# suous/RecNeXt

Measured on AMD Instinct MI355X. Metric: images/sec RecNeXt-M3 224x224 bf16, higher is better.
Workload: dtype bf16

## Files before the change

include/recnext_amd.h:

```cpp
#ifndef RECNEXT_AMD_H
#define RECNEXT_AMD_H

#include <stddef.h>

#ifdef __cplusplus
extern "C" {
#endif

#define RCX_ABI_VERSION 7

enum { RCX_DTYPE_F32 = 0, RCX_DTYPE_BF16 = 1, RCX_DTYPE_F16 = 2 };
enum { RCX_MODE_BILINEAR = 0, RCX_MODE_NEAREST = 1 };
enum { RCX_MAX_LEVEL = 8 };

enum {
    RCX_ERR_BAD_ARG = -1,
    RCX_ERR_UNSUPPORTED = -2,
    RCX_ERR_WORKSPACE = -3
};

int rcx_abi_version(void);
const char* rcx_last_error(void);
void rcx_reload_options(void);

int rcx_selftest_d16(const void* src, void* flag, void* stream);

const char* rcx_recconv2d_fwd_plan(int N, int C, int H, int W, int level, int k, int mode, int dtype);

int rcx_pack_dw_weight(const void* w_ckk, float* dst_kkc, int C, int k, int dtype, void* stream);
int rcx_pack_recconv_params(const void* const* w, const void* const* b, float* wpack, float* wpack_flipped, float* bpack,
                            int count, int C, int k, int dtype, void* stream);
int rcx_unpack_recconv_grads(const float* gwpack, void* const* gw, int count, int C, int k, void* stream);
int rcx_pack_bias(const void* b, float* dst, int C, int dtype, void* stream);

size_t rcx_recconv2d_fwd_workspace_bytes(int N, int C, int H, int W, int level, int k, int dtype);

int rcx_recconv2d_fwd(const void* x, void* y, const float* wpack, const float* bpack,
                      void* workspace, size_t workspace_bytes,
                      int N, int C, int H, int W, int level, int k, int mode, int dtype, void* stream);

int rcx_time_next_launch(void* start_event, void* stop_event);
int rcx_launch_events_pending(void);

size_t rcx_recconv2d_train_saved_bytes(int N, int C, int H, int W, int level, int k);
size_t rcx_recconv2d_bwd_workspace_bytes(int N, int C, int H, int W, int level, int k);
int rcx_recconv2d_fwd_train(const void* x, void* y, const float* wpack, const float* bpack, void* saved, size_t saved_bytes,
                            int N, int C, int H, int W, int level, int k, int mode, int dtype, void* stream);
int rcx_recconv2d_bwd_gy_dtype(int N, int C, int H, int W, int level, int k, int dtype);
const char* rcx_recconv2d_bwd_plan(int N, int C, int H, int W, int level, int k, int dtype);
int rcx_recconv2d_bwd(const void* x, const void* gy, int gy_dtype, const float* wpack, const float* wpack_flipped, const void* saved,
                      void* gx, float* gwpack, float* gbpack, void* const* gw_out, void* const* gb_out, int grad_dtype,
                      void* workspace, size_t workspace_bytes,
                      int N, int C, int H, int W, int level, int k, int mode, int dtype, void* stream);

size_t rcx_recconv2d_bwd_input_workspace_bytes(int N, int C, int H, int W, int level, int k);
int rcx_recconv2d_bwd_input_gy_dtype(int N, int C, int H, int W, int level, int k, int dtype);
const char* rcx_recconv2d_bwd_input_plan(int N, int C, int H, int W, int level, int k, int dtype);
int rcx_recconv2d_bwd_input(const void* gy, int gy_dtype, const float* wpack, const float* wpack_flipped, void* gx,
                            void* workspace, size_t workspace_bytes,
                            int N, int C, int H, int W, int level, int k, int mode, int dtype, void* stream);

int rcx_dwconv2d_fwd(const void* x, void* y, const float* w_kkc, const float* bias,
                     int N, int C, int H, int W, int k, int stride,
                     int in_dtype, int out_dtype, void* stream);

int rcx_dwconv2d_mult2_fwd(const void* x, void* y, const float* w_kkc, const float* bias,
                           int N, int Cin, int H, int W, int k, int stride, int dtype, void* stream);

const char* rcx_upadd_dwconv_fwd_plan(int N, int C, int H, int W, int Hc, int Wc, int k, int mode,
                                      int x_dtype, int coarse_dtype, int out_dtype, int has_coarse);
int rcx_upadd_dwconv_fwd(const void* x, const void* coarse, void* y, const float* w_kkc, const float* bias,
                         int N, int C, int H, int W, int Hc, int Wc, int k, int mode,
                         int x_dtype, int coarse_dtype, int out_dtype, void* stream);

size_t rcx_dwconv2d_bwd_workspace_bytes(int C, int k);
int rcx_dwconv2d_bwd(const void* x, const float* gy, const float* w_kkc, const float* w_flipped_kkc,
                     void* gx, float* gw, float* gb, void* workspace, size_t workspace_bytes,
                     int N, int C, int H, int W, int k, int stride, int x_dtype, void* stream);

size_t rcx_upadd_dwconv_bwd_workspace_bytes(int N, int C, int H, int W, int Hc, int Wc, int k);
int rcx_upadd_dwconv_bwd_gy_dtype(int N, int C, int H, int W, int Hc, int Wc, int k, int dtype);
int rcx_upadd_dwconv_bwd(const void* x, const float* coarse, const void* gy, int gy_dtype, const float* w_kkc, const float* w_flipped_kkc,
                         void* gx, float* gcoarse, float* gw, float* gb, void* workspace, size_t workspace_bytes,
                         int N, int C, int H, int W, int Hc, int Wc, int k, int mode, int dtype, void* stream);

int rcx_dwconv2d_mult2_bwd(const void* x, const float* gy, const float* w_kkc, void* gx, float* gw, float* gb,
                           void* workspace, size_t workspace_bytes, int N, int Cin, int H, int W, int k, int dtype, void* stream);

int rcx_linear_attention_fwd(const void* qpre, const void* kpre, const void* v, const void* pe, void* out,
                             int B, int n, int C, int heads, int dtype, void* stream);
int rcx_linear_attention_pe_fwd(const void* qpre, const void* kpre, const void* v, const float* w_pe_kkc, const float* b_pe, void* out,
                                int B, int H, int W, int C, int heads, int dtype, void* stream);

int rcx_recattn_qkcore_launches(int B, int H, int W, int C, int heads);
size_t rcx_recattn_qkcore_workspace_bytes(int B, int H, int W, int C, int heads);
int rcx_recattn_qkcore_fwd(const float* d, const void* wqk_bf16, const float* bqk, const float* w_pe_kkc, const float* b_pe, float* out,
                           void* workspace, size_t workspace_bytes, int B, int H, int W, int C, int heads, void* stream);

int rcx_recattn_down_qkcore_supported(int B, int H, int W, int C, int heads, int x_dtype);
int rcx_recattn_down_qkcore_fwd(const void* x, const float* w_down_kkc, const float* b_down, const void* wqk_bf16, const float* bqk,
                                const float* w_pe_kkc, const float* b_pe, float* out, int B, int H, int W, int C, int heads, int x_dtype, void* stream);

int rcx_recattn2d_fwd_supported(int B, int H, int W, int C, int heads, int mode, int dtype);
int rcx_recattn2d_fwd(const void* x, void* y, const float* w_down_kkc, const float* b_down, const void* wqk_bf16, const float* bqk,
                      const float* w_pe_kkc, const float* b_pe, const float* w_conv_kkc, const float* b_conv,
                      int B, int H, int W, int C, int heads, int mode, int dtype, void* stream);

int rcx_channel_mlp_supported(int M, int C, int H, int dtype);
size_t rcx_channel_mlp_pack_bytes(int C, int H);
int rcx_channel_mlp_fwd(const void* z, const void* x, void* y, const void* wfrag, const float* bias, int M, int C, int H, int dtype, void* stream);

int rcx_stem_supported(int N, int H, int W, int CM, int CO, int dtype);
size_t rcx_stem_pack_bytes(int CM, int CO);
int rcx_stem_fwd(const void* x, void* y, const void* w1frag, const float* b1, const void* w2frag, const float* b2, int N, int H, int W, int CM, int CO, int dtype, void* stream);

int rcx_stem3_supported(int N, int H, int W, int C, int final_act, int dtype);
size_t rcx_stem3_pack_bytes(int C, int conv);
size_t rcx_stem3_workspace_bytes(int N, int H, int W, int C);
int rcx_stem3_fwd(const void* x, void* y, const void* w1frag, const float* b1, const void* w2frag, const float* b2, const void* w3frag, const float* b3,
                  void* workspace, size_t workspace_bytes, int N, int H, int W, int C, int final_act, int dtype, void* stream);

int rcx_ls_recattn_supported(int B, int H, int W, int C, int split, int heads, int dtype);
int rcx_ls_recattn_fwd(const void* x, void* r, void* t, const float* w_rep, const float* b_rep, const float* w_down_kkc, const float* b_down,
                       const float* wqT, const float* bq, const float* wkT, const float* bk, const float* w_pe_kkc, const float* b_pe,
                       const float* w_conv_kkc, const float* b_conv, int B, int H, int W, int C, int split, int heads, int dtype, void* stream);
int rcx_ls_la3_supported(int B, int H, int W, int C, int split, int heads, int dtype);
int rcx_ls_la3_fwd(const void* x, void* r, void* t, const float* w_rep, const float* b_rep, const float* wqT, const float* bq,
                   const float* wkT, const float* bk, const float* w_pe_kkc, const float* b_pe, int B, int H, int W, int C, int split, int heads,
                   int dtype, void* stream);

int rcx_ls_recattn_tiled_supported(int B, int H, int W, int C, int split, int heads, int dtype);
size_t rcx_ls_recattn_tiled_workspace_bytes(int B, int H, int W, int C, int split, int heads, int dtype);
int rcx_ls_recattn_tiled_fwd(const void* x, void* r, void* t, const float* w_rep, const float* b_rep, const float* w_down_kkc, const float* b_down,
                             const float* wqT, const float* bq, const float* wkT, const float* bk, const float* w_pe_kkc, const float* b_pe,
                             const float* w_conv_kkc, const float* b_conv, void* workspace, size_t workspace_bytes, int B, int H, int W, int C,
                             int split, int heads, int dtype, void* stream);
int rcx_ls_la3_tiled_supported(int B, int H, int W, int C, int split, int heads, int dtype);
size_t rcx_ls_la3_tiled_workspace_bytes(int B, int H, int W, int C, int split, int heads, int dtype);
int rcx_ls_la3_tiled_fwd(const void* x, void* r, void* t, const float* w_rep, const float* b_rep, const float* wqT, const float* bq,
                         const float* wkT, const float* bk, const float* w_pe_kkc, const float* b_pe, void* workspace, size_t workspace_bytes,
                         int B, int H, int W, int C, int split, int heads, int dtype, void* stream);

int rcx_ls_share_supported(int B, int H, int W, int C, int split, int n_src, int dtype);
int rcx_ls_share_fwd(const void* x, void* r, void* t, const float* w_rep, const float* b_rep, const void* const* srcs, int n_src,
                     long long src_pixel_stride, int B, int H, int W, int C, int split, int dtype, void* stream);

int rcx_grouped_conv2d_supported(int N, int H, int W, int Cin, int Cout, int groups, int k, int stride, int dtype);
int rcx_grouped_conv2d_fwd(const void* x, void* y, const float* wpack, const float* bias, int N, int H, int W, int Cin, int Cout, int groups,
                           int k, int stride, int dtype, void* stream);

int rcx_grouped_conv2d_bwd_supported(int N, int H, int W, int Cin, int Cout, int groups, int k, int stride, int dtype);
size_t rcx_grouped_conv2d_bwd_workspace_bytes(int N, int H, int W, int Cin, int Cout, int groups, int k, int stride, int dtype);
int rcx_grouped_conv2d_bwd(const void* x, const void* gy, const float* wpack, void* gx, float* gwpack, float* gb, void* workspace, size_t workspace_bytes,
                           int N, int H, int W, int Cin, int Cout, int groups, int k, int stride, int dtype, void* stream);

int rcx_linear_attention_bwd(const void* qpre, const void* kpre, const void* v, const void* gout, void* gq, void* gk, void* gv,
                             int B, int n, int C, int heads, int dtype, void* stream);

int rcx_linear_attention_wide_supported(int B, int n, int Cqk, int Cv, int heads, int dtype);
int rcx_linear_attention_wide_fwd(const void* qpre, const void* kpre, const void* v, const void* pe, void* out,
                                  int B, int n, int Cqk, int Cv, int heads, int dtype, void* stream);
int rcx_linear_attention_wide_bwd(const void* qpre, const void* kpre, const void* v, const void* gout, void* gq, void* gk, void* gv,
                                  int B, int n, int Cqk, int Cv, int heads, int dtype, void* stream);

int rcx_batchnorm_supported(int N, int H, int W, int C, int dtype);
size_t rcx_batchnorm_workspace_bytes(int N, int H, int W, int C, int dtype);
int rcx_batchnorm_train_fwd(const void* x, void* y, const float* weight, const float* bias, float* running_mean, float* running_var, float* save_mean,
                            float* save_invstd, void* workspace, size_t workspace_bytes, int N, int H, int W, int C, float momentum, float eps, int dtype,
                            void* stream);
int rcx_batchnorm_frozen_fwd(const void* x, void* y, const float* weight, const float* bias, const float* mean, const float* var, float* save_invstd, float eps,
                             int N, int H, int W, int C, int dtype, void* stream);
int rcx_batchnorm_bwd(const void* x, const void* gy, const float* weight, const float* mean, const float* invstd, void* gx, float* gweight, float* gbias,
                      void* workspace, size_t workspace_bytes, int N, int H, int W, int C, int batch_stats, int dtype, void* stream);

int rcx_repdw_train_supported(int N, int H, int W, int C, int dtype);
size_t rcx_repdw_train_workspace_bytes(int N, int H, int W, int C, int dtype);
int rcx_repdw_train_fwd(const void* x, float* r, const float* w3, const float* b3, const float* gamma_a, const float* beta_a, const float* w1, const float* b1,
                        const float* gamma_b, const float* beta_b, float* lk_running_mean, float* lk_running_var, float* sk_running_mean, float* sk_running_var,
                        float* save_mean_x, float* save_var_x, float* save_mean_u, float* save_invstd_u, void* workspace, size_t workspace_bytes,
                        int N, int H, int W, int C, float momentum_a, float eps_a, float momentum_b, float eps_b, int dtype, void* stream);
int rcx_repdw_train_bwd(const void* x, const float* g, const float* w3, const float* b3, const float* gamma_a, const float* w1, const float* gamma_b,
                        const float* mean_x, const float* var_x, const float* mean_u, const float* invstd_u, void* gx, float* gw3, float* gb3, float* ggamma_a,
                        float* gbeta_a, float* gw1, float* gb1, float* ggamma_b, float* gbeta_b, void* workspace, size_t workspace_bytes,
                        int N, int H, int W, int C, float eps_b, int dtype, void* stream);

#ifdef __cplusplus
}
#endif
#endif
```

recnext_amd/_lib.py:

```python
import ctypes
import os

_HERE = os.path.dirname(os.path.abspath(__file__))
LIB_PATH = os.path.join(_HERE, "lib", "librecnext_amd.so")

DTYPE_F32, DTYPE_BF16, DTYPE_F16 = 0, 1, 2
MODE_BILINEAR, MODE_NEAREST = 0, 1
MODES = {"bilinear": MODE_BILINEAR, "nearest": MODE_NEAREST}
MAX_LEVEL = 8
ERR_BAD_ARG, ERR_UNSUPPORTED, ERR_WORKSPACE = -1, -2, -3
ABI_VERSION = 7

_vp, _i, _sz = ctypes.c_void_p, ctypes.c_int, ctypes.c_size_t

SIGNATURES = {
    "rcx_selftest_d16": (_i, [_vp, _vp, _vp]),
    "rcx_abi_version": (_i, []),
    "rcx_last_error": (ctypes.c_char_p, []),
    "rcx_reload_options": (None, []),
    "rcx_recconv2d_fwd_plan": (ctypes.c_char_p, [_i] * 8),
    "rcx_pack_dw_weight": (_i, [_vp, _vp, _i, _i, _i, _vp]),
    "rcx_pack_bias": (_i, [_vp, _vp, _i, _i, _vp]),
    "rcx_pack_recconv_params": (_i, [_vp, _vp, _vp, _vp, _vp, _i, _i, _i, _i, _vp]),
    "rcx_unpack_recconv_grads": (_i, [_vp, _vp, _i, _i, _i, _vp]),
    "rcx_recconv2d_fwd_workspace_bytes": (_sz, [_i] * 7),
    "rcx_recconv2d_fwd": (_i, [_vp, _vp, _vp, _vp, _vp, _sz] + [_i] * 8 + [_vp]),
    "rcx_time_next_launch": (_i, [_vp, _vp]),
    "rcx_launch_events_pending": (_i, []),
    "rcx_recconv2d_train_saved_bytes": (_sz, [_i] * 6),
    "rcx_recconv2d_bwd_workspace_bytes": (_sz, [_i] * 6),
    "rcx_recconv2d_fwd_train": (_i, [_vp, _vp, _vp, _vp, _vp, _sz] + [_i] * 8 + [_vp]),
    "rcx_recconv2d_bwd_gy_dtype": (_i, [_i] * 7),
    "rcx_recconv2d_bwd_plan": (ctypes.c_char_p, [_i] * 7),
    "rcx_upadd_dwconv_bwd_workspace_bytes": (_sz, [_i] * 7),
    "rcx_upadd_dwconv_bwd_gy_dtype": (_i, [_i] * 8),
    "rcx_upadd_dwconv_bwd": (_i, [_vp, _vp, _vp, _i] + [_vp] * 7 + [_sz] + [_i] * 9 + [_vp]),
    "rcx_recconv2d_bwd": (_i, [_vp, _vp, _i] + [_vp] * 8 + [_i, _vp, _sz] + [_i] * 8 + [_vp]),
    "rcx_recconv2d_bwd_input_workspace_bytes": (_sz, [_i] * 6),
    "rcx_recconv2d_bwd_input_gy_dtype": (_i, [_i] * 7),
    "rcx_recconv2d_bwd_input_plan": (ctypes.c_char_p, [_i] * 7),
    "rcx_recconv2d_bwd_input": (_i, [_vp, _i, _vp, _vp, _vp, _vp, _sz] + [_i] * 8 + [_vp]),
    "rcx_dwconv2d_fwd": (_i, [_vp, _vp, _vp, _vp] + [_i] * 8 + [_vp]),
    "rcx_dwconv2d_mult2_fwd": (_i, [_vp, _vp, _vp, _vp] + [_i] * 7 + [_vp]),
    "rcx_upadd_dwconv_fwd": (_i, [_vp, _vp, _vp, _vp, _vp] + [_i] * 11 + [_vp]),
    "rcx_upadd_dwconv_fwd_plan": (ctypes.c_char_p, [_i] * 12),
    "rcx_linear_attention_pe_fwd": (_i, [_vp] * 6 + [_i] * 6 + [_vp]),
    "rcx_recattn_qkcore_launches": (_i, [_i] * 5),
    "rcx_recattn_qkcore_workspace_bytes": (_sz, [_i] * 5),
    "rcx_recattn_qkcore_fwd": (_i, [_vp] * 7 + [_sz] + [_i] * 5 + [_vp]),
    "rcx_recattn_down_qkcore_supported": (_i, [_i] * 6),
    "rcx_recattn_down_qkcore_fwd": (_i, [_vp] * 8 + [_i] * 6 + [_vp]),
    "rcx_stem_supported": (_i, [_i] * 6),
    "rcx_stem_pack_bytes": (_sz, [_i] * 2),
    "rcx_stem_fwd": (_i, [_vp] * 6 + [_i] * 6 + [_vp]),
    "rcx_stem3_supported": (_i, [_i] * 6),
    "rcx_stem3_pack_bytes": (_sz, [_i] * 2),
    "rcx_stem3_workspace_bytes": (_sz, [_i] * 4),
    "rcx_stem3_fwd": (_i, [_vp] * 9 + [_sz] + [_i] * 6 + [_vp]),
    "rcx_channel_mlp_supported": (_i, [_i] * 4),
    "rcx_channel_mlp_pack_bytes": (_sz, [_i] * 2),
    "rcx_channel_mlp_fwd": (_i, [_vp] * 5 + [_i] * 4 + [_vp]),
    "rcx_recattn2d_fwd_supported": (_i, [_i] * 7),
    "rcx_recattn2d_fwd": (_i, [_vp] * 10 + [_i] * 7 + [_vp]),
    "rcx_dwconv2d_bwd_workspace_bytes": (ctypes.c_size_t, [_i, _i]),
    "rcx_dwconv2d_bwd": (_i, [_vp, _vp, _vp, _vp, _vp, _vp, _vp, _vp, ctypes.c_size_t] + [_i] * 7 + [_vp]),
    "rcx_dwconv2d_mult2_bwd": (_i, [_vp, _vp, _vp, _vp, _vp, _vp, _vp, ctypes.c_size_t] + [_i] * 6 + [_vp]),
    "rcx_linear_attention_fwd": (_i, [_vp, _vp, _vp, _vp, _vp] + [_i] * 5 + [_vp]),
    "rcx_ls_recattn_supported": (_i, [_i] * 7),
    "rcx_ls_recattn_fwd": (_i, [_vp] * 15 + [_i] * 7 + [_vp]),
    "rcx_ls_la3_supported": (_i, [_i] * 7),
    "rcx_ls_la3_fwd": (_i, [_vp] * 11 + [_i] * 7 + [_vp]),
    "rcx_ls_recattn_tiled_supported": (_i, [_i] * 7),
    "rcx_ls_recattn_tiled_workspace_bytes": (_sz, [_i] * 7),
    "rcx_ls_recattn_tiled_fwd": (_i, [_vp] * 16 + [_sz] + [_i] * 7 + [_vp]),
    "rcx_ls_la3_tiled_supported": (_i, [_i] * 7),
    "rcx_ls_la3_tiled_workspace_bytes": (_sz, [_i] * 7),
    "rcx_ls_la3_tiled_fwd": (_i, [_vp] * 12 + [_sz] + [_i] * 7 + [_vp]),
    "rcx_grouped_conv2d_supported": (_i, [_i] * 9),
    "rcx_grouped_conv2d_fwd": (_i, [_vp] * 4 + [_i] * 9 + [_vp]),
    "rcx_grouped_conv2d_bwd_supported": (_i, [_i] * 9),
    "rcx_grouped_conv2d_bwd_workspace_bytes": (_sz, [_i] * 9),
    "rcx_grouped_conv2d_bwd": (_i, [_vp] * 7 + [_sz] + [_i] * 9 + [_vp]),
    "rcx_ls_share_supported": (_i, [_i] * 7),
    "rcx_ls_share_fwd": (_i, [_vp] * 6 + [_i, ctypes.c_longlong] + [_i] * 6 + [_vp]),
    "rcx_linear_attention_bwd": (_i, [_vp] * 7 + [_i] * 5 + [_vp]),
    "rcx_linear_attention_wide_supported": (_i, [_i] * 6),
    "rcx_linear_attention_wide_fwd": (_i, [_vp] * 5 + [_i] * 6 + [_vp]),
    "rcx_linear_attention_wide_bwd": (_i, [_vp] * 7 + [_i] * 6 + [_vp]),
    "rcx_batchnorm_supported": (_i, [_i] * 5),
    "rcx_batchnorm_workspace_bytes": (_sz, [_i] * 5),
    "rcx_batchnorm_train_fwd": (_i, [_vp] * 9 + [_sz] + [_i] * 4 + [ctypes.c_float] * 2 + [_i, _vp]),
    "rcx_batchnorm_frozen_fwd": (_i, [_vp] * 7 + [ctypes.c_float] + [_i] * 5 + [_vp]),
    "rcx_batchnorm_bwd": (_i, [_vp] * 9 + [_sz] + [_i] * 6 + [_vp]),
    "rcx_repdw_train_supported": (_i, [_i] * 5),
    "rcx_repdw_train_workspace_bytes": (_sz, [_i] * 5),
    "rcx_repdw_train_fwd": (_i, [_vp] * 19 + [_sz] + [_i] * 4 + [ctypes.c_float] * 4 + [_i, _vp]),
    "rcx_repdw_train_bwd": (_i, [_vp] * 21 + [_sz] + [_i] * 4 + [ctypes.c_float] + [_i, _vp]),
}

_lib = None


class RcxError(RuntimeError):
    pass


def load():
    global _lib
    if _lib is None:
        if not os.path.exists(LIB_PATH):
            raise RcxError(f"{LIB_PATH} not found: build it with `python -c 'import __graft_entry__ as g; g.build()'` "
                           "(or `make -C recnext_amd/csrc`). There is no fallback path.")
        lib = ctypes.CDLL(LIB_PATH)
        for name, (res, args) in SIGNATURES.items():
            fn = getattr(lib, name)
            fn.restype, fn.argtypes = res, args
        got = lib.rcx_abi_version()
        if got != ABI_VERSION:
            raise RcxError(f"librecnext_amd ABI {got} != binding ABI {ABI_VERSION}; rebuild the library")
        _lib = lib
    return _lib


def check(rc, what):
    if rc != 0:
        msg = load().rcx_last_error().decode("utf-8", "replace")
        raise RcxError(f"{what} failed (code {rc}): {msg}")
```

recnext_amd/csrc/rcx_api.hip:

```cpp
#include "../../include/recnext_amd.h"
#include "rcx_opts.h"
#include "rcx_launch.h"

#include <cstdarg>
#include <initializer_list>
#include <cstdio>
#include <cstdlib>

namespace {

thread_local char g_err[512] = "";

int fail(int code, const char* fmt, ...)
{
    va_list ap;
    va_start(ap, fmt);
    vsnprintf(g_err, sizeof(g_err), fmt, ap);
    va_end(ap);
    return code;
}

int hip_fail(hipError_t e, const char* what, const char* prefix = "")
{
    snprintf(g_err, sizeof(g_err), "%s%s: %s", prefix, what, hipGetErrorString(e));
// ... 929 lines not shown
                                         "in fours (2, 4 or 8 heads), where the LDS holds the plane (rcx_recattn_qkcore_launches; use the projection GEMMs + "
                                         "rcx_linear_attention_pe_fwd)", C / heads, heads, H * W, C);
    const size_t need = rcx::recattn_qkcore_workspace_bytes(B, H, W, C, heads);
    if (need && (!workspace || workspace_bytes < need || ((size_t)workspace & 15)))
        return fail(RCX_ERR_WORKSPACE, "rcx_recattn_qkcore_fwd: needs a 16-byte-aligned workspace of %zu bytes, got %zu", need, workspace ? workspace_bytes : (size_t)0);
    hipError_t e = rcx::recattn_qkcore(d, wqk_bf16, bqk, w_pe_kkc, b_pe, out, workspace, B, H, W, C, heads, (hipStream_t)stream);
    return e == hipSuccess ? 0 : hip_fail(e, "rcx_recattn_qkcore_fwd");
}

int rcx_recattn_down_qkcore_supported(int B, int H, int W, int C, int heads, int x_dtype)
{
    if (B <= 0 || H <= 0 || W <= 0 || C <= 0 || heads <= 0 || C % heads) return 0;
    return rcx::recattn_down_qkcore_applicable(B, H, W, C, heads, x_dtype) ? 1 : 0;
}

int rcx_recattn_down_qkcore_fwd(const void* x, const float* w_down_kkc, const float* b_down, const void* wqk_bf16, const float* bqk,
                                const float* w_pe_kkc, const float* b_pe, float* out, int B, int H, int W, int C, int heads, int x_dtype, void* stream)
{
    if (!x || !w_down_kkc || !wqk_bf16 || !bqk || !w_pe_kkc || !out) return fail(RCX_ERR_BAD_ARG, "rcx_recattn_down_qkcore_fwd: null pointer");
    if (B <= 0 || H <= 0 || W <= 0 || C <= 0 || heads <= 0) return fail(RCX_ERR_BAD_ARG, "non-positive extent B=%d H=%d W=%d C=%d heads=%d", B, H, W, C, heads);
    if (C % heads) return fail(RCX_ERR_BAD_ARG, "C=%d is not a multiple of heads=%d", C, heads);
    if (!known_dtype(x_dtype)) return fail(RCX_ERR_BAD_ARG, "unknown dtype %d", x_dtype);
    if (((size_t)wqk_bf16 & 15) || ((size_t)out & 15) || ((size_t)bqk & 15) || ((size_t)w_pe_kkc & 15) || ((size_t)b_pe & 15))
        return fail(RCX_ERR_BAD_ARG, "rcx_recattn_down_qkcore_fwd: wqk, bqk, w_pe_kkc, b_pe and out must be 16-byte aligned");
    if (!rcx::recattn_down_qkcore_applicable(B, H, W, C, heads, x_dtype))
        return fail(RCX_ERR_UNSUPPORTED, "rcx_recattn_down_qkcore_fwd: %d x %d plane, %d heads of %d, dtype %d: the one-launch form takes the 14 x 14 plane (1 .. 8 heads) "
                                         "and the 7 x 7 plane (1 .. 16 heads) of bf16 / f16 activations, heads of 4 .. 32 channels, or 2, 4 or 8 heads of 36 .. 64 in fours "
                                         "whose image fits the LDS (use rcx_dwconv2d_fwd + rcx_recattn_qkcore_fwd)",
                    H, W, heads, C / heads, x_dtype);
    hipError_t e = rcx::recattn_down_qkcore(x, w_down_kkc, b_down, wqk_bf16, bqk, w_pe_kkc, b_pe, out, B, H, C, heads, x_dtype, (hipStream_t)stream);
    return e == hipSuccess ? 0 : hip_fail(e, "rcx_recattn_down_qkcore_fwd");
}

int rcx_recattn2d_fwd_supported(int B, int H, int W, int C, int heads, int mode, int dtype)
{
    if (B <= 0 || H <= 0 || W <= 0 || C <= 0 || heads <= 0 || C % heads) return 0;
    return rcx::recattn2d_unit_applicable(B, H, W, C, heads, dtype, mode == RCX_MODE_NEAREST ? 1 : 0) ? 1 : 0;
}

int rcx_recattn2d_fwd(const void* x, void* y, const float* w_down_kkc, const float* b_down, const void* wqk_bf16, const float* bqk,
                      const float* w_pe_kkc, const float* b_pe, const float* w_conv_kkc, const float* b_conv,
                      int B, int H, int W, int C, int heads, int mode, int dtype, void* stream)
{
    if (!x || !y || !w_down_kkc || !wqk_bf16 || !bqk || !w_pe_kkc || !w_conv_kkc) return fail(RCX_ERR_BAD_ARG, "rcx_recattn2d_fwd: null pointer");
    if (B <= 0 || H <= 0 || W <= 0 || C <= 0 || heads <= 0) return fail(RCX_ERR_BAD_ARG, "non-positive extent B=%d H=%d W=%d C=%d heads=%d", B, H, W, C, heads);
    if (C % heads) return fail(RCX_ERR_BAD_ARG, "C=%d is not a multiple of heads=%d", C, heads);
    if (!known_dtype(dtype)) return fail(RCX_ERR_BAD_ARG, "unknown dtype %d", dtype);
    if (mode != RCX_MODE_BILINEAR && mode != RCX_MODE_NEAREST) return fail(RCX_ERR_BAD_ARG, "unknown mode %d", mode);
    if (((size_t)wqk_bf16 & 15) || ((size_t)bqk & 15) || ((size_t)w_pe_kkc & 15) || ((size_t)b_pe & 15))
        return fail(RCX_ERR_BAD_ARG, "rcx_recattn2d_fwd: wqk, bqk, w_pe_kkc and b_pe must be 16-byte aligned");
    if (!rcx::recattn2d_unit_applicable(B, H, W, C, heads, dtype, mode == RCX_MODE_NEAREST ? 1 : 0))
        return fail(RCX_ERR_UNSUPPORTED, "rcx_recattn2d_fwd: %d x %d plane, %d heads of %d, mode %d, dtype %d: the one-launch unit takes the 14 x 14 (1 .. 8 heads) and 7 x 7 (1 .. 16 heads) planes of bf16 / f16 "
                                         "activations, heads of 32 or 4 .. 28 channels (not above 32), nearest resize (use rcx_recattn_down_qkcore_fwd / rcx_dwconv2d_fwd + rcx_recattn_qkcore_fwd, then "
                                         "rcx_upadd_dwconv_fwd)", H, W, heads, C / heads, mode, dtype);
    hipError_t e = rcx::recattn2d_unit(x, w_down_kkc, b_down, wqk_bf16, bqk, w_pe_kkc, b_pe, w_conv_kkc, b_conv, y, B, H, C, heads, dtype, (hipStream_t)stream);
    return e == hipSuccess ? 0 : hip_fail(e, "rcx_recattn2d_fwd");
}

int rcx_stem_supported(int N, int H, int W, int CM, int CO, int dtype) { return rcx::stem_applicable(N, H, W, CM, CO, dtype) ? 1 : 0; }

size_t rcx_stem_pack_bytes(int CM, int CO) { return rcx::stem_pack_bytes(CM, CO); }

int rcx_stem_fwd(const void* x, void* y, const void* w1frag, const float* b1, const void* w2frag, const float* b2, int N, int H, int W, int CM, int CO, int dtype, void* stream)
{
    if (!x || !y || !w1frag || !b1 || !w2frag || !b2) return fail(RCX_ERR_BAD_ARG, "rcx_stem_fwd: null pointer");
    if (N <= 0 || H <= 0 || W <= 0 || CM <= 0 || CO <= 0) return fail(RCX_ERR_BAD_ARG, "non-positive extent N=%d H=%d W=%d CM=%d CO=%d", N, H, W, CM, CO);
    if (!known_dtype(dtype)) return fail(RCX_ERR_BAD_ARG, "unknown dtype %d", dtype);
    if (((size_t)x & 1) || ((size_t)y & 7) || ((size_t)w1frag & 15) || ((size_t)b1 & 15) || ((size_t)w2frag & 15) || ((size_t)b2 & 15))
        return fail(RCX_ERR_BAD_ARG, "rcx_stem_fwd: w1frag, b1, w2frag and b2 must be 16-byte aligned, y 8-byte aligned");
    if (!rcx::stem_applicable(N, H, W, CM, CO, dtype))
        return fail(RCX_ERR_UNSUPPORTED, "rcx_stem_fwd: no kernel for CM=%d CO=%d dtype %d (bf16; CM in {20, 24, 28, 32, 40}, CO %% 4 == 0, CO <= 96; one image of x below 2^31 bytes)", CM, CO, dtype);
    hipError_t e = rcx::stem_fwd(x, y, w1frag, b1, w2frag, b2, N, H, W, CM, CO, dtype, (hipStream_t)stream);
    return e == hipSuccess ? 0 : hip_fail(e, "rcx_stem_fwd");
}

namespace {
bool stem3_shape(int N, int H, int W, int C, int final_act, int dtype)
{
    if (dtype != RCX_DTYPE_BF16 || N <= 0 || H <= 0 || W <= 0 || (C != 64 && C != 128) || (final_act != 0 && final_act != 1)) return false;
    if ((unsigned long long)H * W * 6 >= (1ull << 31)) return false;
    const long long h2 = ((H + 1) / 2 + 1) / 2, w2 = ((W + 1) / 2 + 1) / 2;
    return (long long)N * h2 * w2 <= 0x7fffffffLL / 64;
}
bool any_misaligned(std::initializer_list<const void*> ps)
{
    for (const void* p : ps)
        if ((size_t)p & 15) return true;
    return false;
}
bool overlap(const void* a, size_t na, const void* b, size_t nb)
{
    return (const char*)a < (const char*)b + nb && (const char*)b < (const char*)a + na;
}
}

int rcx_stem3_supported(int N, int H, int W, int C, int final_act, int dtype) { return stem3_shape(N, H, W, C, final_act, dtype) ? 1 : 0; }

size_t rcx_stem3_pack_bytes(int C, int conv)
{
    if (C != 64 && C != 128) return 0;
    if (conv == 1) return 2048;
    if (conv == 2) return (size_t)(C / 64) * 9 * ((C / 4 + 15) / 16) * 1024;
    if (conv == 3) return (size_t)(C / 32) * 9 * (C / 32) * 1024;
    return 0;
}

size_t rcx_stem3_workspace_bytes(int N, int H, int W, int C)
{
    if (N <= 0 || H <= 0 || W <= 0 || (C != 64 && C != 128)) return 0;
    return (size_t)N * (size_t)(((H + 1) / 2 + 1) / 2) * (size_t)(((W + 1) / 2 + 1) / 2) * (size_t)(C / 2) * 2;
}

int rcx_stem3_fwd(const void* x, void* y, const void* w1frag, const float* b1, const void* w2frag, const float* b2, const void* w3frag, const float* b3,
                  void* workspace, size_t workspace_bytes, int N, int H, int W, int C, int final_act, int dtype, void* stream)
{
    if (!x || !y || !w1frag || !b1 || !w2frag || !b2 || !w3frag || !b3 || !workspace) return fail(RCX_ERR_BAD_ARG, "rcx_stem3_fwd: null pointer");
    if (N <= 0 || H <= 0 || W <= 0 || C <= 0) return fail(RCX_ERR_BAD_ARG, "non-positive extent N=%d H=%d W=%d C=%d", N, H, W, C);
    if (!known_dtype(dtype)) return fail(RCX_ERR_BAD_ARG, "unknown dtype %d", dtype);
    if (final_act != 0 && final_act != 1) return fail(RCX_ERR_BAD_ARG, "rcx_stem3_fwd: final_act must be 0 or 1, got %d", final_act);
    if (((size_t)x & 1) || any_misaligned({y, workspace, w1frag, b1, w2frag, b2, w3frag, b3}))
        return fail(RCX_ERR_BAD_ARG, "rcx_stem3_fwd: y, workspace and the six packs must be 16-byte aligned, x 2-byte aligned");
    if (!stem3_shape(N, H, W, C, final_act, dtype))
        return fail(RCX_ERR_UNSUPPORTED, "rcx_stem3_fwd: no kernel for C=%d dtype %d (bf16; C = 64 | 128; one image of x below 2^31 bytes)", C, dtype);
    const size_t need = rcx_stem3_workspace_bytes(N, H, W, C), xbytes = (size_t)N * H * W * 6;
    const size_t ybytes = (size_t)N * (size_t)((((H + 1) / 2 + 1) / 2 + 1) / 2) * (size_t)((((W + 1) / 2 + 1) / 2 + 1) / 2) * (size_t)C * 2;
    if (overlap(y, ybytes, x, xbytes) || overlap(workspace, workspace_bytes, x, xbytes) || overlap(workspace, workspace_bytes, y, ybytes))
        return fail(RCX_ERR_BAD_ARG, "rcx_stem3_fwd: y and the workspace must overlap neither x nor each other");
    if (workspace_bytes < need) return fail(RCX_ERR_WORKSPACE, "rcx_stem3_fwd: needs a workspace of %zu bytes, got %zu", need, workspace_bytes);
    hipError_t e = rcx::stem_front_fwd(x, workspace, w1frag, b1, w2frag, b2, N, H, W, C / 4, (hipStream_t)stream);
    if (e != hipSuccess) return hip_fail(e, "rcx_stem3_fwd (front)");
    e = rcx::conv3s2_fwd(workspace, y, w3frag, b3, N, ((H + 1) / 2 + 1) / 2, ((W + 1) / 2 + 1) / 2, C / 2, final_act, (hipStream_t)stream);
    return e == hipSuccess ? 0 : hip_fail(e, "rcx_stem3_fwd (tail)");
}

int rcx_channel_mlp_supported(int M, int C, int H, int dtype) { return rcx::channel_mlp_applicable(M, C, H, dtype) ? 1 : 0; }

size_t rcx_channel_mlp_pack_bytes(int C, int H) { return rcx::channel_mlp_pack_bytes(C, H); }

int rcx_channel_mlp_fwd(const void* z, const void* x, void* y, const void* wfrag, const float* bias, int M, int C, int H, int dtype, void* stream)
{
    if (!z || !x || !y || !wfrag || !bias) return fail(RCX_ERR_BAD_ARG, "rcx_channel_mlp_fwd: null pointer");
    if (M <= 0 || C <= 0 || H <= 0) return fail(RCX_ERR_BAD_ARG, "non-positive extent M=%d C=%d H=%d", M, C, H);
    if (!known_dtype(dtype)) return fail(RCX_ERR_BAD_ARG, "unknown dtype %d", dtype);
    if (((size_t)z & 15) || ((size_t)x & 7) || ((size_t)y & 7) || ((size_t)wfrag & 15) || ((size_t)bias & 15))
        return fail(RCX_ERR_BAD_ARG, "rcx_channel_mlp_fwd: z, wfrag and bias must be 16-byte aligned, x and y 8-byte aligned");
    if (y == z || y == x) return fail(RCX_ERR_BAD_ARG, "rcx_channel_mlp_fwd: y must not alias its inputs");
    if (!rcx::channel_mlp_applicable(M, C, H, dtype))
        return fail(RCX_ERR_UNSUPPORTED, "rcx_channel_mlp_fwd: no kernel for M=%d C=%d H=%d dtype %d (bf16; (C, H) = (40 | 48, 96), (56 | 64, 128), (80, 160), (96, 192), (128, 256), (160, 320), "
                                         "(192, 384), (256, 512), (320, 640), and (384, 768), (512, 768), (512, 1024) each from a minimum M upward; M C 2 < 2^31)", M, C, H, dtype);
    hipError_t e = rcx::channel_mlp(z, x, y, wfrag, bias, M, C, H, dtype, (hipStream_t)stream);
    return e == hipSuccess ? 0 : hip_fail(e, "rcx_channel_mlp_fwd");
}

int rcx_ls_recattn_supported(int B, int H, int W, int C, int split, int heads, int dtype)
{
    return rcx::ls_recattn_applicable(B, H, W, C, split, heads, dtype) ? 1 : 0;
}

int rcx_ls_la3_supported(int B, int H, int W, int C, int split, int heads, int dtype)
{
    return rcx::ls_la3_applicable(B, H, W, C, split, heads, dtype) ? 1 : 0;
}

int rcx_ls_recattn_fwd(const void* x, void* r, void* t, const float* w_rep, const float* b_rep, const float* w_down_kkc, const float* b_down,
                       const float* wqT, const float* bq, const float* wkT, const float* bk, const float* w_pe_kkc, const float* b_pe,
                       const float* w_conv_kkc, const float* b_conv, int B, int H, int W, int C, int split, int heads, int dtype, void* stream)
{
    if (!x || !r || !t || !w_rep || !b_rep || !w_down_kkc || !b_down || !wqT || !bq || !wkT || !bk || !w_pe_kkc || !b_pe || !w_conv_kkc || !b_conv)
        return fail(RCX_ERR_BAD_ARG, "rcx_ls_recattn_fwd: null pointer");
    if (B <= 0 || H <= 0 || W <= 0 || C <= 0 || split <= 0 || heads <= 0)
        return fail(RCX_ERR_BAD_ARG, "non-positive extent B=%d H=%d W=%d C=%d split=%d heads=%d", B, H, W, C, split, heads);
    if (!known_dtype(dtype)) return fail(RCX_ERR_BAD_ARG, "unknown dtype %d", dtype);
    if (r == x || t == x || r == t) return fail(RCX_ERR_BAD_ARG, "rcx_ls_recattn_fwd: r and t must alias neither x nor each other");
    if (any_misaligned({x, r, t, w_rep, b_rep, w_down_kkc, b_down, wqT, bq, wkT, bk, w_pe_kkc, b_pe, w_conv_kkc, b_conv}))
        return fail(RCX_ERR_BAD_ARG, "rcx_ls_recattn_fwd: every tensor must be 16-byte aligned");
    if (!rcx::ls_recattn_applicable(B, H, W, C, split, heads, dtype))
        return fail(RCX_ERR_UNSUPPORTED, "rcx_ls_recattn_fwd: %d x %d plane, C=%d, split=%d, %d heads: one head, C and split multiples of 4, and an image whose slice "
                                         "mixer fits the LDS", H, W, C, split, heads);
    hipError_t e = rcx::ls_recattn_fwd(x, r, t, w_rep, b_rep, w_down_kkc, b_down, wqT, bq, wkT, bk, w_pe_kkc, b_pe, w_conv_kkc, b_conv,
                                       B, H, W, C, split, dtype, (hipStream_t)stream);
    return e == hipSuccess ? 0 : hip_fail(e, "rcx_ls_recattn_fwd");
}

int rcx_ls_la3_fwd(const void* x, void* r, void* t, const float* w_rep, const float* b_rep, const float* wqT, const float* bq,
                   const float* wkT, const float* bk, const float* w_pe_kkc, const float* b_pe, int B, int H, int W, int C, int split, int heads,
                   int dtype, void* stream)
{
    if (!x || !r || !t || !w_rep || !b_rep || !wqT || !bq || !wkT || !bk || !w_pe_kkc || !b_pe) return fail(RCX_ERR_BAD_ARG, "rcx_ls_la3_fwd: null pointer");
    if (B <= 0 || H <= 0 || W <= 0 || C <= 0 || split <= 0 || heads <= 0)
        return fail(RCX_ERR_BAD_ARG, "non-positive extent B=%d H=%d W=%d C=%d split=%d heads=%d", B, H, W, C, split, heads);
    if (!known_dtype(dtype)) return fail(RCX_ERR_BAD_ARG, "unknown dtype %d", dtype);
    if (r == x || t == x || r == t) return fail(RCX_ERR_BAD_ARG, "rcx_ls_la3_fwd: r and t must alias neither x nor each other");
    if (any_misaligned({x, r, t, w_rep, b_rep, wqT, bq, wkT, bk, w_pe_kkc, b_pe}))
        return fail(RCX_ERR_BAD_ARG, "rcx_ls_la3_fwd: every tensor must be 16-byte aligned");
    if (!rcx::ls_la3_applicable(B, H, W, C, split, heads, dtype))
        return fail(RCX_ERR_UNSUPPORTED, "rcx_ls_la3_fwd: %d x %d plane, C=%d, split=%d, %d heads: at most 64 tokens, C and split multiples of 4, split a multiple "
                                         "of 2 heads", H, W, C, split, heads);
    hipError_t e = rcx::ls_la3_fwd(x, r, t, w_rep, b_rep, wqT, bq, wkT, bk, w_pe_kkc, b_pe, B, H, W, C, split, heads, dtype, (hipStream_t)stream);
    return e == hipSuccess ? 0 : hip_fail(e, "rcx_ls_la3_fwd");
}

int rcx_ls_recattn_tiled_supported(int B, int H, int W, int C, int split, int heads, int dtype)
{
    return rcx::ls_recattn_tiled_applicable(B, H, W, C, split, heads, dtype) ? 1 : 0;
}

int rcx_ls_la3_tiled_supported(int B, int H, int W, int C, int split, int heads, int dtype)
{
    return rcx::ls_la3_tiled_applicable(B, H, W, C, split, heads, dtype) ? 1 : 0;
}

size_t rcx_ls_recattn_tiled_workspace_bytes(int B, int H, int W, int C, int split, int heads, int dtype)
{
    return rcx::ls_recattn_tiled_workspace_bytes(B, H, W, C, split, heads, dtype);
}

size_t rcx_ls_la3_tiled_workspace_bytes(int B, int H, int W, int C, int split, int heads, int dtype)
{
    return rcx::ls_la3_tiled_workspace_bytes(B, H, W, C, split, heads, dtype);
}

namespace {
int check_ls_tiled(const char* fn, std::initializer_list<const void*> ps, const void* x, const void* r, const void* t, const void* workspace,
                   size_t workspace_bytes, size_t need, bool supported, int B, int H, int W, int C, int split, int heads, int dtype)
{
    for (const void* p : ps)
        if (!p) return fail(RCX_ERR_BAD_ARG, "%s: null pointer", fn);
    if (B <= 0 || H <= 0 || W <= 0 || C <= 0 || split <= 0 || heads <= 0)
        return fail(RCX_ERR_BAD_ARG, "non-positive extent B=%d H=%d W=%d C=%d split=%d heads=%d", B, H, W, C, split, heads);
    if (!known_dtype(dtype)) return fail(RCX_ERR_BAD_ARG, "unknown dtype %d", dtype);
    if (r == x || t == x || r == t) return fail(RCX_ERR_BAD_ARG, "%s: r and t must alias neither x nor each other", fn);
    if (workspace && (workspace == x || workspace == r || workspace == t)) return fail(RCX_ERR_BAD_ARG, "%s: the workspace must alias none of x, r and t", fn);
    if (any_misaligned(ps) || ((size_t)workspace & 15)) return fail(RCX_ERR_BAD_ARG, "%s: every tensor and the workspace must be 16-byte aligned", fn);
    if (!supported)
        return fail(RCX_ERR_UNSUPPORTED, "%s: %d x %d plane, C=%d, split=%d, %d heads: C and split multiples of 4; RecAttn2d one head, LinearAttention3 split a "
                                         "multiple of 2 heads with heads of v in fours; a chunk's LDS within 160 KB", fn, H, W, C, split, heads);
    if (!workspace || workspace_bytes < need) return fail(RCX_ERR_WORKSPACE, "%s: workspace of %zu bytes, %zu needed", fn, workspace_bytes, need);
    return 0;
}
}

int rcx_ls_recattn_tiled_fwd(const void* x, void* r, void* t, const float* w_rep, const float* b_rep, const float* w_down_kkc, const float* b_down,
                             const float* wqT, const float* bq, const float* wkT, const float* bk, const float* w_pe_kkc, const float* b_pe,
                             const float* w_conv_kkc, const float* b_conv, void* workspace, size_t workspace_bytes, int B, int H, int W, int C,
                             int split, int heads, int dtype, void* stream)
{
    if (int rc = check_ls_tiled("rcx_ls_recattn_tiled_fwd", {x, r, t, w_rep, b_rep, w_down_kkc, b_down, wqT, bq, wkT, bk, w_pe_kkc, b_pe, w_conv_kkc, b_conv},
                                x, r, t, workspace, workspace_bytes, rcx::ls_recattn_tiled_workspace_bytes(B, H, W, C, split, heads, dtype),
                                rcx::ls_recattn_tiled_applicable(B, H, W, C, split, heads, dtype), B, H, W, C, split, heads, dtype))
        return rc;
    hipError_t e = rcx::ls_recattn_tiled_fwd(x, r, t, w_rep, b_rep, w_down_kkc, b_down, wqT, bq, wkT, bk, w_pe_kkc, b_pe, w_conv_kkc, b_conv, workspace,
                                             B, H, W, C, split, dtype, (hipStream_t)stream);
    return e == hipSuccess ? 0 : hip_fail(e, "rcx_ls_recattn_tiled_fwd");
}

int rcx_ls_la3_tiled_fwd(const void* x, void* r, void* t, const float* w_rep, const float* b_rep, const float* wqT, const float* bq,
                         const float* wkT, const float* bk, const float* w_pe_kkc, const float* b_pe, void* workspace, size_t workspace_bytes,
                         int B, int H, int W, int C, int split, int heads, int dtype, void* stream)
{
    if (int rc = check_ls_tiled("rcx_ls_la3_tiled_fwd", {x, r, t, w_rep, b_rep, wqT, bq, wkT, bk, w_pe_kkc, b_pe}, x, r, t, workspace, workspace_bytes,
                                rcx::ls_la3_tiled_workspace_bytes(B, H, W, C, split, heads, dtype),
                                rcx::ls_la3_tiled_applicable(B, H, W, C, split, heads, dtype), B, H, W, C, split, heads, dtype))
        return rc;
    hipError_t e = rcx::ls_la3_tiled_fwd(x, r, t, w_rep, b_rep, wqT, bq, wkT, bk, w_pe_kkc, b_pe, workspace, B, H, W, C, split, heads, dtype,
                                         (hipStream_t)stream);
    return e == hipSuccess ? 0 : hip_fail(e, "rcx_ls_la3_tiled_fwd");
}

int rcx_grouped_conv2d_supported(int N, int H, int W, int Cin, int Cout, int groups, int k, int stride, int dtype)
{
    return rcx::ls_down_applicable(N, H, W, Cin, Cout, groups, k, stride, dtype) ? 1 : 0;
}

int rcx_grouped_conv2d_fwd(const void* x, void* y, const float* wpack, const float* bias, int N, int H, int W, int Cin, int Cout, int groups, int k,
                           int stride, int dtype, void* stream)
{
    if (!x || !y || !wpack) return fail(RCX_ERR_BAD_ARG, "rcx_grouped_conv2d_fwd: null pointer");
    if (N <= 0 || H <= 0 || W <= 0 || Cin <= 0 || Cout <= 0 || groups <= 0)
        return fail(RCX_ERR_BAD_ARG, "rcx_grouped_conv2d_fwd: non-positive extent N=%d H=%d W=%d Cin=%d Cout=%d groups=%d", N, H, W, Cin, Cout, groups);
    if (!known_dtype(dtype)) return fail(RCX_ERR_BAD_ARG, "rcx_grouped_conv2d_fwd: unknown dtype %d", dtype);
    if (y == x || (const void*)wpack == x || (const void*)wpack == y || (bias && ((const void*)bias == x || (const void*)bias == y)))
        return fail(RCX_ERR_BAD_ARG, "rcx_grouped_conv2d_fwd: y must alias neither x nor a pack");
    const size_t es = dtype == RCX_DTYPE_F32 ? 4 : 2;
    if ((size_t)x % es || (size_t)y % es || (size_t)wpack % 4 || (size_t)bias % 4)
        return fail(RCX_ERR_BAD_ARG, "rcx_grouped_conv2d_fwd: x and y must be aligned to one element (%zu bytes), the packs to 4 bytes", es);
    if (!rcx::ls_down_applicable(N, H, W, Cin, Cout, groups, k, stride, dtype))
        return fail(RCX_ERR_UNSUPPORTED, "rcx_grouped_conv2d_fwd: Cin=%d, Cout=%d, groups=%d, k=%d, stride=%d: k = 5, stride = 2, groups dividing Cin and Cout, "
                                         "1 .. 4 channels a group in and out, fewer than 2^31 elements in x and in y", Cin, Cout, groups, k, stride);
    hipError_t e = rcx::ls_down_fwd(x, y, wpack, bias, N, H, W, Cin, Cout, groups, dtype, (hipStream_t)stream);
    return e == hipSuccess ? 0 : hip_fail(e, "rcx_grouped_conv2d_fwd");
}

int rcx_grouped_conv2d_bwd_supported(int N, int H, int W, int Cin, int Cout, int groups, int k, int stride, int dtype)
{
    return rcx::ls_down_bwd_applicable(N, H, W, Cin, Cout, groups, k, stride, dtype) ? 1 : 0;
}

size_t rcx_grouped_conv2d_bwd_workspace_bytes(int N, int H, int W, int Cin, int Cout, int groups, int k, int stride, int dtype)
{
    return rcx::ls_down_bwd_workspace_bytes(N, H, W, Cin, Cout, groups, k, stride, dtype);
}

int rcx_grouped_conv2d_bwd(const void* x, const void* gy, const float* wpack, void* gx, float* gwpack, float* gb, void* workspace, size_t workspace_bytes,
                           int N, int H, int W, int Cin, int Cout, int groups, int k, int stride, int dtype, void* stream)
{
    if (!x || !gy || !wpack) return fail(RCX_ERR_BAD_ARG, "rcx_grouped_conv2d_bwd: null pointer");
// ... 268 lines not shown
```

recnext_amd/csrc/rcx_launch.h:

```cpp
#pragma once
#include <hip/hip_runtime.h>
#include <hip/hip_ext.h>
#include <stddef.h>

#include <atomic>
#define RCX_MAX_DEVICES 64
#define RCX_SET_LDS_ONCE(kfn, bytes)                                                                                              \
    do {                                                                                                                          \
        static std::atomic<size_t> rcx_lds_set_[RCX_MAX_DEVICES];                                                                 \
        int rcx_dev_ = 0;                                                                                                         \
        if (hipGetDevice(&rcx_dev_) != hipSuccess || rcx_dev_ < 0 || rcx_dev_ >= RCX_MAX_DEVICES) rcx_dev_ = RCX_MAX_DEVICES - 1; \
        if ((size_t)(bytes) > 64 * 1024 && (size_t)(bytes) > rcx_lds_set_[rcx_dev_].load(std::memory_order_acquire)) {            \
            hipError_t rcx_e_ = hipFuncSetAttribute(reinterpret_cast<const void*>(kfn), hipFuncAttributeMaxDynamicSharedMemorySize, (int)(bytes)); \
            if (rcx_e_ != hipSuccess) return rcx_e_;                                                                              \
            if (rcx_dev_ != RCX_MAX_DEVICES - 1) rcx_lds_set_[rcx_dev_].store((size_t)(bytes), std::memory_order_release);        \
        }                                                                                                                         \
    } while (0)

namespace rcx {

struct LaunchEvents { hipEvent_t start = nullptr, stop = nullptr; };
LaunchEvents take_launch_events();
#define RCX_LAUNCH_TIMED(kfn, grid, block, lds, stream, ...)                                                                       \
    do {                                                                                                                           \
        const rcx::LaunchEvents rcx_ev_ = rcx::take_launch_events();                                                               \
        if (rcx_ev_.start || rcx_ev_.stop) hipExtLaunchKernelGGL(kfn, grid, block, lds, stream, rcx_ev_.start, rcx_ev_.stop, 0, __VA_ARGS__); \
        else hipLaunchKernelGGL(kfn, grid, block, lds, stream, __VA_ARGS__);                                                       \
    } while (0)

hipError_t generic_dwconv(const void* x, void* y, const float* w, const float* b,
                          int N, int C, int H, int W, int k, int stride, int in_dt, int out_dt, hipStream_t s);
hipError_t generic_upadd_dwconv(const void* x, const void* coarse, void* y, const float* w, const float* b,
                                int N, int C, int H, int W, int Hc, int Wc, int k, int mode,
                                int x_dt, int c_dt, int out_dt, hipStream_t s);
hipError_t generic_dwconv_mult2(const void* x, void* y, const float* w, const float* b,
                                int N, int Cin, int H, int W, int k, int stride, int dt, hipStream_t s);
hipError_t pack_dw_weight(const void* w, float* dst, int C, int k, int dt, hipStream_t s);
hipError_t selftest_d16(const void* src, void* flag, hipStream_t s);
hipError_t pack_bias(const void* b, float* dst, int C, int dt, hipStream_t s);
struct PackPtrs { const void* w[10]; const void* b[10]; };
hipError_t pack_params(const PackPtrs& P, float* wpack, float* wflip, float* bpack, int count, int C, int k, int dt, hipStream_t s);
hipError_t unpack_grads(const float* gwpack, const PackPtrs& P, int count, int C, int k, hipStream_t s);

bool plane_applicable(int N, int C, int H, int W, int level, int k, int dtype);
int plane_describe(int N, int C, int H, int W, int level, int k, int dtype, char* buf, int len);
hipError_t plane_recconv(const void* x, void* y, const float* wpack, const float* bpack,
                         int N, int C, int H, int W, int level, int k, int mode, int dtype, hipStream_t s);

bool lanes_applicable(int N, int C, int H, int W, int level, int k, int dtype);
int lanes_describe(int N, int C, int H, int W, int level, int k, int mode, int dtype, char* buf, int len);
hipError_t lanes_recconv(const void* x, void* y, const float* wpack, const float* bpack,
                         int N, int C, int H, int W, int level, int k, int mode, int dtype, hipStream_t s);

hipError_t lanes16_recconv(const void* x, void* y, const float* wpack, const float* bpack,
                           int N, int C, int H, int W, int level, int k, int mode, int dtype, hipStream_t s);


bool cpl14_applicable(int N, int C, int H, int W, int level, int k, int dtype);
bool cpl14_short_applicable(int N, int C, int H, int W, int level, int k, int dtype);
int cpl14_short_describe(int N, int C, int mode, char* buf, int len);
hipError_t cpl14_short_recconv(const void* x, void* y, const float* wpack, const float* bpack, int N, int C, int mode, int dtype, hipStream_t s);
int cpl14_describe(int N, int C, int mode, int dtype, char* buf, int len);
hipError_t cpl14_recconv(const void* x, void* y, const float* wpack, const float* bpack, int N, int C, int mode, int dtype, hipStream_t s,
                         float* saved = nullptr, const size_t* f_off = nullptr, const size_t* c_off = nullptr);

bool upadd_cpt_applicable(int N, int C, int H, int W, int Hc, int Wc, int k, int x_dt, int c_dt, int out_dt);
int upadd_cpt_describe(int N, int C, int H, int W, int mode, int x_dt, char* buf, int len);
hipError_t upadd_cpt(const void* x, const void* coarse, void* y, const float* w, const float* b, int N, int C, int H, int W, int mode,
                     int x_dt, int c_dt, hipStream_t s);
bool down7m2_cpt_applicable(int N, int Cin, int H, int W, int k, int stride, int dtype);
hipError_t down7m2_cpt(const void* x, void* y, const float* w, const float* b, int N, int Cin, int H, int W, int dtype, hipStream_t s);
bool down5_cpt_applicable(int N, int C, int H, int W, int k, int stride, int in_dt, int out_dt);
hipError_t down5_cpt(const void* x, void* y, const float* w, const float* b, int N, int C, int H, int W, int in_dt, int out_dt, hipStream_t s);
bool upadd_cpl14_applicable(int N, int C, int H, int W, int Hc, int Wc, int k, int x_dt, int c_dt, int out_dt);
hipError_t upadd_cpl14(const void* x, const void* coarse, void* y, const float* w, const float* b, int N, int C, int H, int mode, int x_dt, int c_dt,
                       hipStream_t s);
bool down5_cpl7_applicable(int N, int C, int H, int W, int k, int stride, int in_dt, int out_dt);
hipError_t down5_cpl7(const void* x, void* y, const float* w, const float* b, int N, int C, int H, int in_dt, hipStream_t s);

bool cpl7b_applicable(int N, int C, int H, int W, int level, int k, int dtype);
int cpl7b_describe(int N, int C, int mode, char* buf, int len);
hipError_t cpl7b_recconv(const void* x, void* y, const float* wpack, const float* bpack, int N, int C, int mode, int dtype, hipStream_t s,
                         float* saved = nullptr, const size_t* f_off = nullptr, const size_t* c_off = nullptr);

bool cplbwd_applicable(int N, int C, int H, int W, int level, int k, int dtype);
bool cplbwd_split(int N, int C);
hipError_t cplbwd_recconv(const void* x, const void* gy, const float* wpack, const float* wflip, const void* saved,
                          const size_t* f_off, const size_t* c_off, void* gx, float* const* part,
                          int N, int C, int H, int level, int mode, int dtype, hipStream_t s, int gy_dt = 0);

bool cpladj_applicable(int N, int C, int H, int W, int level, int k, int dtype);
hipError_t cpladj_recconv(const void* gy, int gy_dt, const float* wpack, const float* wflip, void* gx, int gx_dt, int N, int C, int H, int mode,
                          hipStream_t s);

bool wgrad_cpl_applicable(int N, int C, int H, int W, int Hc, int Wc, int k, int stride, bool has_coarse);
hipError_t wgrad_cpl(const void* a, int a_dt, const float* coarse, const void* g, int g_dt, float* partial, int N, int C, int H, int mode,
                     hipStream_t s, int* rows_out);

bool wgrad2_cpl_applicable(int N, int C, int H, int W, int Ho, int Wo, int k, int stride, bool has_coarse);
hipError_t wgrad2_cpl(const void* a, int a_dt, const float* g, float* partial, int N, int C, int H, hipStream_t s, int* rows_out);
bool wgrad2m_cpl_applicable(int N, int Cout, int H, int W, int k);
hipError_t wgrad2m_cpl(const void* a, int a_dt, const float* g, float* partial, int N, int Cout, int H, hipStream_t s, int* rows_out);

bool bwd_cpt_applicable(int N, int C, int H, int W, int k);
hipError_t bwd_gc_cpt(const void* g, int g_dt, float* gC, const float* wf, int N, int C, int H, int mode, hipStream_t s);
bool bwd_wgrad_dm_cpt_applicable(int N, int Cout, int H, int W, int k);
hipError_t bwd_wgrad_dm_cpt(const void* a, int a_dt, const float* G, float* partial, int N, int Cout, int H, hipStream_t s, int* rows_out);
bool bwd_down7m2_cpt_applicable(int N, int Cin, int H, int W, int k);
hipError_t bwd_down7m2_cpt(const float* g, void* gx, int x_dt, const float* w, int N, int Cin, int H, hipStream_t s);
hipError_t bwd_wgrad_k_cpt(const void* a, int a_dt, const float* coarse, const void* g, int g_dt, float* partial, int N, int C, int H, int mode, hipStream_t s,
                           int* rows_out);
hipError_t bwd_wgrad_d_cpt(const void* a, int a_dt, const float* G, float* partial, int N, int C, int H, hipStream_t s, int* rows_out);
hipError_t bwd_dT_cpt(const float* G, void* out, int out_dt, const float* wd, int N, int C, int H, hipStream_t s);
hipError_t bwd_gx_cpt(const void* g, int g_dt, const float* G, void* out, int out_dt, const float* wf, const float* wd, int N, int C, int H, hipStream_t s);

bool cpt_applicable(int N, int C, int H, int W, int level, int k, int dtype);
int cpt_describe(int N, int C, int H, int level, int mode, int dtype, char* buf, int len);
bool cpt_train_applicable(int N, int C, int H, int W, int level, int k, int mode, int dtype);
hipError_t cpt_recconv(const void* x, void* y, const float* wpack, const float* bpack, int N, int C, int H, int level, int mode, int dtype, hipStream_t s,
                       float* saved = nullptr, const size_t* f_off = nullptr, const size_t* c_off = nullptr);
bool down_lanes_applicable(int N, int Cin, int H, int W, int k, int stride, int dtype);
hipError_t down_lanes(const void* x, void* y, const float* w, const float* b, int N, int Cin, int H, int W, int k, int stride, int dtype, hipStream_t s);

bool upadd_lanes_applicable(int N, int C, int H, int W, int Hc, int Wc, int k, int x_dt, int c_dt, int out_dt);
hipError_t upadd_lanes(const void* x, const void* coarse, void* y, const float* w, const float* b,
                       int N, int C, int H, int W, int mode, int x_dt, int c_dt, hipStream_t s);
bool conv5_lanes_applicable(int N, int C, int H, int W, int k, int x_dt, int out_dt);
hipError_t conv5_lanes(const void* x, void* y, const float* w, const float* b, int N, int C, int H, int W, int x_dt, hipStream_t s);
bool down5_lanes_applicable(int N, int C, int H, int W, int k, int stride, int in_dt, int out_dt);
hipError_t down5_lanes(const void* x, void* y, const float* w, const float* b, int N, int C, int H, int W, int in_dt, int out_dt, hipStream_t s);

hipError_t linattn_core(const void* qpre, const void* kpre, const void* v, const void* pe, void* out,
                        int B, int n, int C, int heads, int dtype, hipStream_t s, const float* pew = nullptr, const float* peb = nullptr, int Wp = 0);
bool linattn_core_fuses_pe(int n, int C, int heads, int dtype);
bool recattn_qkcore_applicable(int B, int Hp, int Wp, int C, int heads);
int recattn_qkcore_launches(int B, int Hp, int Wp, int C, int heads);
size_t recattn_qkcore_workspace_bytes(int B, int Hp, int Wp, int C, int heads);
bool recattn_down_qkcore_applicable(int B, int H, int W, int C, int heads, int x_dt);
hipError_t recattn_down_qkcore(const void* x, const float* wdn, const float* bdn, const void* wqk_bf16, const float* bqk, const float* wpe, const float* bpe,
                               float* out, int B, int H, int C, int heads, int x_dt, hipStream_t s);
bool stem_applicable(int N, int H, int W, int CM, int CO, int dtype);
size_t stem_pack_bytes(int CM, int CO);
hipError_t stem_fwd(const void* x, void* y, const void* w1frag, const float* b1, const void* w2frag, const float* b2, int N, int H, int W, int CM, int CO, int dtype, hipStream_t s);
int stem_device_cus();
hipError_t stem_front_fwd(const void* x, void* y, const void* w1frag, const float* b1, const void* w2frag, const float* b2, int N, int H, int W, int CM, hipStream_t s);
hipError_t conv3s2_fwd(const void* x, void* y, const void* wfrag, const float* bias, int N, int H, int W, int CIN, int act, hipStream_t s);
bool channel_mlp_applicable(int M, int C, int H, int dtype);
size_t channel_mlp_pack_bytes(int C, int H);
hipError_t channel_mlp(const void* z, const void* x, void* y, const void* wfrag, const float* bias, int M, int C, int H, int dtype, hipStream_t s);
bool recattn2d_unit_applicable(int B, int H, int W, int C, int heads, int x_dt, int mode);
hipError_t recattn2d_unit(const void* x, const float* wdn, const float* bdn, const void* wqk_bf16, const float* bqk, const float* wpe, const float* bpe,
                          const float* wcv, const float* bcv, void* y, int B, int H, int C, int heads, int x_dt, hipStream_t s);
bool ls_recattn_applicable(int B, int H, int W, int C, int split, int heads, int dtype);
bool ls_la3_applicable(int B, int H, int W, int C, int split, int heads, int dtype);
hipError_t ls_recattn_fwd(const void* x, void* r, void* t, const float* w_rep, const float* b_rep, const float* w_dn, const float* b_dn,
                          const float* wqT, const float* bq, const float* wkT, const float* bk, const float* w_pe, const float* b_pe,
                          const float* w_cv, const float* b_cv, int B, int H, int W, int C, int split, int dtype, hipStream_t s);
hipError_t ls_la3_fwd(const void* x, void* r, void* t, const float* w_rep, const float* b_rep, const float* wqT, const float* bq,
                      const float* wkT, const float* bk, const float* w_pe, const float* b_pe, int B, int H, int W, int C, int split, int heads,
                      int dtype, hipStream_t s);
bool ls_recattn_tiled_applicable(int B, int H, int W, int C, int split, int heads, int dtype);
bool ls_la3_tiled_applicable(int B, int H, int W, int C, int split, int heads, int dtype);
size_t ls_recattn_tiled_workspace_bytes(int B, int H, int W, int C, int split, int heads, int dtype);
size_t ls_la3_tiled_workspace_bytes(int B, int H, int W, int C, int split, int heads, int dtype);
hipError_t ls_recattn_tiled_fwd(const void* x, void* r, void* t, const float* w_rep, const float* b_rep, const float* w_dn, const float* b_dn,
                                const float* wqT, const float* bq, const float* wkT, const float* bk, const float* w_pe, const float* b_pe,
                                const float* w_cv, const float* b_cv, void* workspace, int B, int H, int W, int C, int split, int dtype, hipStream_t s);
hipError_t ls_la3_tiled_fwd(const void* x, void* r, void* t, const float* w_rep, const float* b_rep, const float* wqT, const float* bq,
                            const float* wkT, const float* bk, const float* w_pe, const float* b_pe, void* workspace, int B, int H, int W, int C,
                            int split, int heads, int dtype, hipStream_t s);
constexpr int kLsShareMaxSrc = 8;
bool ls_share_applicable(int B, int H, int W, int C, int split, int n_src, long long stride, int dtype);
hipError_t ls_share_fwd(const void* x, void* r, void* t, const float* w_rep, const float* b_rep, const void* const* srcs, int n_src, long long stride,
                        int B, int H, int W, int C, int split, int dtype, hipStream_t s);
bool ls_down_applicable(int N, int H, int W, int Cin, int Cout, int groups, int k, int stride, int dtype);
hipError_t ls_down_fwd(const void* x, void* y, const float* wpack, const float* bias, int N, int H, int W, int Cin, int Cout, int groups, int dtype,
                       hipStream_t s);
bool ls_down_bwd_applicable(int N, int H, int W, int Cin, int Cout, int groups, int k, int stride, int dtype);
size_t ls_down_bwd_workspace_bytes(int N, int H, int W, int Cin, int Cout, int groups, int k, int stride, int dtype);
hipError_t ls_down_bwd(const void* x, const void* gy, const float* wpack, void* gx, float* gw, float* gb, void* workspace, int N, int H, int W, int Cin,
                       int Cout, int groups, int dtype, hipStream_t s);
bool batchnorm_applicable(long long N, long long H, long long W, long long C, int dtype);
size_t batchnorm_workspace_bytes(int R, int C, int dtype);
hipError_t batchnorm_train_fwd(const void* x, void* y, const float* weight, const float* bias, float* run_mean, float* run_var, float* save_mean,
                               float* save_invstd, void* workspace, int R, int C, float momentum, float eps, int dtype, hipStream_t s);
hipError_t batchnorm_frozen_fwd(const void* x, void* y, const float* weight, const float* bias, const float* mean, const float* var, float* save_invstd,
                                int R, int C, float eps, int dtype, hipStream_t s);
hipError_t batchnorm_bwd(const void* x, const void* gy, const float* weight, const float* mean, const float* invstd, void* gx, float* gweight, float* gbias,
                         void* workspace, int R, int C, bool batch_stats, int dtype, hipStream_t s);
size_t repdw_train_workspace_bytes(int R, int C, int dtype);
hipError_t repdw_train_fwd(const void* x, float* out, const float* w3, const float* b3, const float* gamma_a, const float* beta_a, const float* w1, const float* b1,
                           const float* gamma_b, const float* beta_b, float* lk_rm, float* lk_rv, float* sk_rm, float* sk_rv, float* mean_x, float* var_x,
                           float* mean_u, float* invstd_u, void* workspace, int N, int H, int W, int C, float mom_a, float eps_a, float mom_b, float eps_b,
                           int dtype, hipStream_t s);
hipError_t repdw_train_bwd(const void* x, const float* g, const float* w3, const float* b3, const float* gamma_a, const float* w1, const float* gamma_b,
                           const float* mean_x, const float* var_x, const float* mean_u, const float* invstd_u, void* gx, float* gw3, float* gb3, float* ggamma_a,
                           float* gbeta_a, float* gw1, float* gb1, float* ggamma_b, float* gbeta_b, void* workspace, int N, int H, int W, int C, float eps_b,
                           int dtype, hipStream_t s);
hipError_t recattn_qkcore(const float* d,const void* wqk_bf16, const float* bqk, const float* wpe, const float* bpe, float* out, void* workspace,
                          int B, int Hp, int Wp, int C, int heads, hipStream_t s);

hipError_t linattn_core_bwd(const void* qpre, const void* kpre, const void* v, const void* gout, void* gq, void* gk, void* gv,
                            int B, int n, int C, int heads, int dtype, hipStream_t s);
bool linattn_wide_applicable(int B, int n, int Cqk, int Cv, int heads, int dtype);
hipError_t linattn_wide_fwd(const void* qpre, const void* kpre, const void* v, const void* pe, void* out, int B, int n, int Cqk, int Cv, int heads,
                            int dtype, hipStream_t s);
hipError_t linattn_wide_bwd(const void* qpre, const void* kpre, const void* v, const void* gout, void* gq, void* gk, void* gv, int B, int n, int Cqk,
                            int Cv, int heads, int dtype, hipStream_t s);

size_t wgrad_partial_bytes(int C, int k);
hipError_t bwd_wgrad(const void* a, int a_dt, const float* coarse, const float* g, float* partial, float* gw, float* gb,
                     int N, int C, int H, int W, int Hc, int Wc, int Ho, int Wo, int k, int stride, int mode, int accumulate, hipStream_t s,
                     int* rows_out = nullptr,
                     int g_dt = 0);
struct WgradJobs {
    int njobs, kk, C;
    int nslots[10];
    int rows[10][8];
    const float* part[10][8];
    float* gw[10];
    float* gb[10];
    int param_layout, param_dt;
};
hipError_t bwd_wgrad_reduce_jobs(const WgradJobs& J, hipStream_t s);
hipError_t bwd_mult2(const void* x, int x_dt, const float* g, const float* w, void* gx, float* partial, float* gw, float* gb,
                     int N, int Cin, int H, int W, int k, hipStream_t s);
hipError_t bwd_down_input(const float* base, const float* g, void* out, int out_dt, const float* w,
                          int N, int C, int H, int W, int Hc, int Wc, int k, hipStream_t s);
hipError_t bwd_resize(const float* gfine, float* gcoarse, int N, int C, int H, int W, int Hc, int Wc, int mode, hipStream_t s);

}
```

recnext_amd/csrc/rcx_mlp.hip:

```cpp
#include "rcx_common.h"
#include "rcx_launch.h"
#include "rcx_gelu.h"
#include <type_traits>

#ifdef RCX_MLP_STAMPS
#define RCX_MLP_STAMP(k)                                                                                        \
    {                                                                                                           \
        __builtin_amdgcn_sched_barrier(0);                                                                      \
        unsigned long long t_;                                                                                  \
        asm volatile("s_memtime %0\n\ts_waitcnt lgkmcnt(0)" : "=s"(t_)::"memory");                              \
        __builtin_amdgcn_sched_barrier(0);                                                                      \
        tsum[k] += t_ - tlast;                                                                                  \
        tlast = t_;                                                                                             \
    }
#define RCX_MLP_STAMP_BEGIN                                                                                     \
    unsigned long long tsum[7] = {0, 0, 0, 0, 0, 0, 0}, tlast;                                                  \
    asm volatile("s_memtime %0\n\ts_waitcnt lgkmcnt(0)" : "=s"(tlast)::"memory");
#define RCX_MLP_STAMP_STEP tsum[6] += 1;
#define RCX_MLP_STAMP_END(slot)                                                                                 \
    if (stamps && (threadIdx.x & 63) == 0) {                                                                    \
        _Pragma("unroll") for (int k_ = 0; k_ < 7; ++k_) stamps[(size_t)(slot) * 8 + k_] = tsum[k_];            \
    }
#define RCX_MLP_STAMP_PARM , unsigned long long (&tsum)[7], unsigned long long& tlast
#define RCX_MLP_STAMP_PASS , tsum, tlast
#define RCX_MLP_STAMP_ARG , unsigned long long* __restrict__ stamps
#define RCX_MLP_STAMP_VAL , g_stamps
namespace rcx {
static unsigned long long* g_stamps = nullptr;
}
#else
#define RCX_MLP_STAMP(k)
#define RCX_MLP_STAMP_BEGIN
#define RCX_MLP_STAMP_STEP
#define RCX_MLP_STAMP_END(slot)
#define RCX_MLP_STAMP_PARM
#define RCX_MLP_STAMP_PASS
#define RCX_MLP_STAMP_ARG
#define RCX_MLP_STAMP_VAL
#endif

#ifndef RCX_MLP_PINNED
#define RCX_MLP_PINNED true
#endif

namespace rcx {
namespace mlp {

typedef float f32x16 __attribute__((ext_vector_type(16)));
typedef float f32x4q __attribute__((ext_vector_type(4)));
typedef float f32x2q __attribute__((ext_vector_type(2)));
typedef __bf16 bf16x8 __attribute__((ext_vector_type(8)));
typedef __bf16 bf16x4 __attribute__((ext_vector_type(4)));
typedef unsigned u32x4q __attribute__((ext_vector_type(4)));
typedef unsigned u32x2q __attribute__((ext_vector_type(2)));

__device__ __forceinline__ void wave_sync()
{
    __builtin_amdgcn_fence(__ATOMIC_RELEASE, "wavefront");
    __builtin_amdgcn_wave_barrier();
    __builtin_amdgcn_fence(__ATOMIC_ACQUIRE, "wavefront");
}


__device__ __forceinline__ __amdgpu_buffer_rsrc_t token_rows(const void* p, unsigned nbytes) { return __builtin_amdgcn_make_buffer_rsrc((void*)p, 0, nbytes, 0x00020000); }

#define RCX_MLP_ZERO(D, N)                                                                                                                \
    _Pragma("unroll") for (int n_ = 0; n_ < N; ++n_) _Pragma("unroll") for (int i_ = 0; i_ < 16; ++i_) D[n_][i_] = 0.f;

#define RCX_MLP_STAGE_Z(ZA)                                                                                                               \
    _Pragma("unroll") for (int q = 0; q < ZH; ++q) {                                                                                      \
        _Pragma("unroll") for (int i = 0; i < KH; ++i) *reinterpret_cast<u32x4q*>(Lt + (ZA)) = zq[q * KH + i];                            \
        wave_sync();                                                                                                                      \
        _Pragma("unroll") for (int k = 0; k < KH; ++k)                                                                                    \
            zb[q * KH + k] = __builtin_bit_cast(bf16x8, *reinterpret_cast<const u32x4q*>(Lt + r * ZP + 32 * k + 16 * h));                 \
        wave_sync();                                                                                                                      \
    }

#define RCX_MLP_IMAGE_QUAD(D2, B2, DST)                                                                                                   \
    {                                                                                                                                     \
        const f32x4q bb = *reinterpret_cast<const f32x4q*>(B2);                                                                           \
        *reinterpret_cast<f32x4q*>(DST) = f32x4q{D2[4 * g] + bb.x, D2[4 * g + 1] + bb.y, D2[4 * g + 2] + bb.z, D2[4 * g + 3] + bb.w};     \
    }

__device__ __forceinline__ bf16x8 rows_plus_x(f32x4q lo, f32x4q hi, u32x4q xv)
{
    bf16x8 o;
    o[0] = (__bf16)(lo.x + __uint_as_float(xv.x << 16)); o[1] = (__bf16)(lo.y + __uint_as_float(xv.x & 0xffff0000u));
    o[2] = (__bf16)(lo.z + __uint_as_float(xv.y << 16)); o[3] = (__bf16)(lo.w + __uint_as_float(xv.y & 0xffff0000u));
    o[4] = (__bf16)(hi.x + __uint_as_float(xv.z << 16)); o[5] = (__bf16)(hi.y + __uint_as_float(xv.z & 0xffff0000u));
    o[6] = (__bf16)(hi.z + __uint_as_float(xv.w << 16)); o[7] = (__bf16)(hi.w + __uint_as_float(xv.w & 0xffff0000u));
    return o;
}

constexpr int imax(int a, int b) { return a > b ? a : b; }
constexpr size_t bias_bytes(int HT, int CT) { return sizeof(float) * 32 * (HT + CT); }

template <int KS1, int HT, int CT, int NW, bool STAGED>
struct SmallLds {
    static constexpr int NF = HT * (KS1 + 2 * CT), ZP = 32 * KS1 + 16, OP = 128 * CT + 16, IMG = STAGED ? 32 * imax(ZP, OP) : 0;
    static constexpr size_t b1 = (size_t)NF * 1024, images = b1 + bias_bytes(HT, CT), bytes = images + (size_t)NW * IMG;
};
template <int KS1, int HT, int CT, int NW, int ZH>
struct StreamLds {
    static constexpr int NCH = KS1 + 2 * CT, ZP = 32 * KS1 / ZH + 16, OP = 256 + 16, IMG = 32 * imax(ZP, OP);
    static constexpr size_t b1 = (size_t)2 * NCH * 1024, images = b1 + bias_bytes(HT, CT), bytes = images + (size_t)NW * IMG;
};
template <int KS1, int HT, int CT>
struct PairLds {
    static constexpr int NW = 8, NS = 3, ZH = 4, NCH = KS1 + 2 * CT, ZP = 32 * KS1 / ZH + 16, OP = 128 + 16, IMG = 32 * imax(ZP, OP);
    static constexpr size_t b1 = (size_t)NS * NCH * 1024, images = b1 + bias_bytes(HT, CT), bytes = images + (size_t)NW * IMG;
};
template <int KS1, int HT, int CT>
struct Res128Lds {
    static constexpr int NW = 8, ZH = 4, NCH = KS1 + 2 * CT, NF = HT * NCH, ZP = 32 * KS1 / ZH + 16, OC = 16, OP = 4 * OC + 16, IMG = 32 * imax(ZP, OP);
    static constexpr size_t b1 = (size_t)NF * 1024, images = b1 + bias_bytes(HT, CT), bytes = images + (size_t)NW * IMG;
};
template <int KS1, int HT, int CT, int NW>
struct WideLds {
    static constexpr int ZBYTES = 2 * KS1 * 1024, XBYTES = NW * 4 * 1024, OP = 256 + 16, IMG = 32 * OP;
    static constexpr size_t xchg = ZBYTES, b1 = (size_t)ZBYTES + 2 * XBYTES, bytes = b1 + bias_bytes(HT, CT);
    static_assert(NW * IMG <= ZBYTES + XBYTES, "the output images alias the z fragments and exchange buffer 0");
};

#define RCX_MLP_HIDDEN_GELU(D1, QUAD)                                                                                                     \
    bf16x8 hb[2];                                                                                                                         \
    gelu_f32x2 gv[8];                                                                                                                     \
    _Pragma("unroll") for (int g = 0; g < 4; ++g) {                                                                                       \
        const f32x4q bb = QUAD;                                                                                                           \
        gv[2 * g] = gelu_f32x2{D1[4 * g] + bb.x, D1[4 * g + 1] + bb.y};                                                                   \
        gv[2 * g + 1] = gelu_f32x2{D1[4 * g + 2] + bb.z, D1[4 * g + 3] + bb.w};                                                           \
    }                                                                                                                                     \
    {                                                                                                                                     \
        gelu_f32x2 ga[4] = {gv[0], gv[1], gv[2], gv[3]}, gb[4] = {gv[4], gv[5], gv[6], gv[7]};                                            \
        gelu2x_batch<4>(ga);                                                                                                              \
        gelu2x_batch<4>(gb);                                                                                                              \
        _Pragma("unroll") for (int i = 0; i < 4; ++i) { gv[i] = ga[i]; gv[4 + i] = gb[i]; }                                               \
    }                                                                                                                                     \
    _Pragma("unroll") for (int g = 0; g < 4; ++g) {                                                                                       \
        hb[g >> 1][4 * (g & 1) + 0] = (__bf16)gv[2 * g].x; hb[g >> 1][4 * (g & 1) + 1] = (__bf16)gv[2 * g].y;                             \
        hb[g >> 1][4 * (g & 1) + 2] = (__bf16)gv[2 * g + 1].x; hb[g >> 1][4 * (g & 1) + 3] = (__bf16)gv[2 * g + 1].y;                     \
    }

template <int KS1, int CT, int RD>
__device__ __forceinline__ void hidden_tile_ring(const u32x4q* Lc, const float* b1t, int lane, int h, const bf16x8 (&zb)[KS1], f32x16 (&d2)[CT] RCX_MLP_STAMP_PARM)
{
    constexpr int R1 = KS1 < RD ? KS1 : RD, N2 = 2 * CT, R2 = N2 < RD ? N2 : RD;
    u32x4q ring[RD];
#pragma unroll
    for (int j = 0; j < R1; ++j) ring[j] = Lc[j * 64 + lane];
    RCX_MLP_STAMP(0)
    f32x16 d1;
#pragma unroll
    for (int i = 0; i < 16; ++i) d1[i] = 0.f;
#pragma unroll
    for (int ks = 0; ks < KS1; ++ks) {
// ... 320 lines not shown
        const u32x4q* src = wfrag + (size_t)chunk * NCH * 64 + threadIdx.x;
        u32x4q* dst = Lring + (size_t)slot * NCH * 64 + wv * 64;
        if constexpr (PIN) {
            const unsigned l0 = (unsigned)(size_t)(__attribute__((address_space(3))) void*)dst;
            unsigned m0_;
#pragma unroll
            for (int i = 0; i < PER; ++i)
                asm volatile("s_mov_b32 %0, m0\n\ts_mov_b32 m0, %2\n\ts_nop 0\n\tglobal_load_lds_dwordx4 %1, off\n\ts_mov_b32 m0, %0" : "=&s"(m0_) : "v"(src + i * NT), "s"(l0 + 16u * i * NT) : "memory");
        } else {
#pragma unroll
            for (int i = 0; i < PER; ++i)
                __builtin_amdgcn_global_load_lds((__attribute__((address_space(1))) void*)(src + i * NT), (__attribute__((address_space(3))) void*)(dst + i * NT), 16, 0, 0);
        }
    };
    constexpr int VM_ALL = 0x70, VM_NEXT = 0x70 | (PER & 15) | ((PER >> 4) << 14);
    fill(0, 0);
    fill(1, 1);
    for (int i = threadIdx.x; i < 32 * (HT + CT); i += NT) Lb1[i] = bias[i];
    const unsigned nbytes = (unsigned)M * (unsigned)C * 2u;
    const __amdgpu_buffer_rsrc_t zsrc = token_rows(z, nbytes), xsrc = token_rows(xres, nbytes), ysrc = token_rows(y, nbytes);
    const unsigned zo0 = (unsigned)(lane >> 3) * RB + 16u * (lane & 7), za0 = (unsigned)(lane >> 3) * ZP + 16u * (lane & 7);
    const unsigned ot = lane >> 2, ob = 16u * (lane & 3);
    if (!(__builtin_popcount(wv) & 1)) __builtin_amdgcn_s_setprio(1);
    RCX_MLP_STAMP_BEGIN
    int slot = 0;
    for (int block = blockIdx.x; block < nblocks; block += gridDim.x) {
        const unsigned base = (unsigned)(32 * (block * NW + wave)) * (unsigned)RB;
        const bool more = block + (int)gridDim.x < nblocks;
        bf16x8 zb[KS1];
        {
            u32x4q zq[KS1];
#pragma unroll
            for (int i = 0; i < KS1; ++i)
                zq[i] = __builtin_bit_cast(u32x4q, __builtin_amdgcn_raw_buffer_load_b128(zsrc, (int)(base + zo0 + 8u * RB * (i % KH) + RBH * (i / KH)), 0, 0));
            RCX_MLP_STAGE_Z(za0 + 8 * ZP * i)
        }
        f32x16 d2[CT];
        RCX_MLP_ZERO(d2, CT)
        RCX_MLP_STAMP(5)
#pragma unroll 1
        for (int ht = 0; ht < HT; ++ht) {
            if (ht + 1 < HT || more) __builtin_amdgcn_s_waitcnt(VM_NEXT);
            else __builtin_amdgcn_s_waitcnt(VM_ALL);
            __builtin_amdgcn_s_barrier();
            if (ht + 2 < HT || more) fill((ht + 2) % HT, slot == 0 ? 2 : slot - 1);
            RCX_MLP_STAMP(4)
            if constexpr (PIN) {
                hidden_tile_pinned<KS1, CT, 4, 1, 3>(Lring + (size_t)slot * NCH * 64, Lb1 + 32 * ht, lane, h, zb, d2 RCX_MLP_STAMP_PASS);
            } else
                hidden_tile_ring<KS1, CT, 4>(Lring + (size_t)slot * NCH * 64, Lb1 + 32 * ht, lane, h, zb, d2 RCX_MLP_STAMP_PASS);
            RCX_MLP_STAMP_STEP
            slot = slot == NS - 1 ? 0 : slot + 1;
        }
        u32x4q xq[CT][2];
#pragma unroll
        for (int ct = 0; ct < CT; ++ct)
#pragma unroll
            for (int j = 0; j < 2; ++j)
                xq[ct][j] = __builtin_bit_cast(u32x4q, __builtin_amdgcn_raw_buffer_load_b128(xsrc, (int)(base + (16u * j + ot) * RB + 64u * ct + ob), 0, 0));
#pragma unroll
        for (int ct = 0; ct < CT; ++ct) {
#pragma unroll
            for (int g = 0; g < 4; ++g) RCX_MLP_IMAGE_QUAD(d2[ct], Lb2 + 32 * ct + 8 * g + 4 * h, Lt + r * OP + 4 * (8 * g + 4 * h))
            wave_sync();
#pragma unroll
            for (int j = 0; j < 2; ++j) {
                const unsigned char* src = Lt + (16 * j + ot) * OP + 2 * ob;
                const f32x4q lo = *reinterpret_cast<const f32x4q*>(src), hi = *reinterpret_cast<const f32x4q*>(src + 16);
                __builtin_amdgcn_raw_buffer_store_b128(__builtin_bit_cast(u32x4q, rows_plus_x(lo, hi, xq[ct][j])), ysrc, (int)(base + (16u * j + ot) * RB + 64u * ct + ob), 0, 0);
            }
            wave_sync();
        }
    }
    RCX_MLP_STAMP(5)
    RCX_MLP_STAMP_END(blockIdx.x * NW + wv)
}


template <int KS1, int HT, int CT>
__global__ void __launch_bounds__(512, 2)
k_channel_mlp_res128(const bf16_t* __restrict__ z, const bf16_t* __restrict__ xres, bf16_t* __restrict__ y, const u32x4q* __restrict__ wfrag, const float* __restrict__ bias,
                     int M, int ntiles RCX_MLP_STAMP_ARG)
{
    extern __shared__ __attribute__((aligned(16))) unsigned char lds_raw[];
    using L = Res128Lds<KS1, HT, CT>;
    constexpr int NW = L::NW, NT = 64 * NW, NCH = L::NCH, NF = L::NF, PER = NF * 64 / NT;
    static_assert(NF * 64 % NT == 0, "whole pieces per wave");
    constexpr int ZH = L::ZH, RB = 32 * KS1, RBH = RB / ZH, KH = KS1 / ZH, ZP = L::ZP;
    static_assert(KS1 % ZH == 0 && RBH == 64, "column parts of 32 channels: a request = 16 token rows of 64 bytes");
    constexpr int OC = L::OC, NP = 32 * CT / OC, OP = L::OP;
    const u32x4q* const Lf = reinterpret_cast<const u32x4q*>(lds_raw);
    float* const Lb1 = reinterpret_cast<float*>(lds_raw + L::b1);
    const float* const Lb2 = Lb1 + 32 * HT;
    const int lane = threadIdx.x & 63, r = lane & 31, h = lane >> 5;
    const int wv = __builtin_amdgcn_readfirstlane(threadIdx.x >> 6);
    unsigned char* const Lt = lds_raw + L::images + (size_t)wv * L::IMG;
    {
        const u32x4q* src = wfrag + threadIdx.x;
        u32x4q* dst = reinterpret_cast<u32x4q*>(lds_raw) + wv * 64;
#pragma unroll
        for (int i = 0; i < PER; ++i)
            __builtin_amdgcn_global_load_lds((__attribute__((address_space(1))) void*)(src + i * NT), (__attribute__((address_space(3))) void*)(dst + i * NT), 16, 0, 0);
        for (int i = threadIdx.x; i < 32 * (HT + CT); i += NT) Lb1[i] = bias[i];
    }
    const unsigned nbytes = (unsigned)M * (unsigned)RB;
    const __amdgpu_buffer_rsrc_t zsrc = token_rows(z, nbytes), xsrc = token_rows(xres, nbytes), ysrc = token_rows(y, nbytes);
    const unsigned zo0 = (unsigned)(lane >> 2) * RB + 16u * (lane & 3), za0 = (unsigned)(lane >> 2) * ZP + 16u * (lane & 3);
    const unsigned ot = lane / 2, ob = 16u * (lane % 2);
    const int stride = NW * (int)gridDim.x;
    int tile = wv * (int)gridDim.x + (int)blockIdx.x;
    u32x4q zq[KS1];
    auto load_z = [&](int t) {
        const unsigned base = (unsigned)t * 32u * RB;
#pragma unroll
        for (int i = 0; i < KS1; ++i)
            zq[i] = __builtin_bit_cast(u32x4q, __builtin_amdgcn_raw_buffer_load_b128(zsrc, (int)(base + zo0 + 16u * RB * (i % KH) + RBH * (i / KH)), 0, 0));
    };
    if (tile < ntiles) load_z(tile);
    __builtin_amdgcn_s_waitcnt(0x70);
    __syncthreads();
    RCX_MLP_STAMP_BEGIN
    for (; tile < ntiles; tile += stride) {
        const unsigned base = (unsigned)tile * 32u * RB;
        bf16x8 zb[KS1];
        RCX_MLP_STAGE_Z(za0 + 16 * ZP * i)
        if (tile + stride < ntiles) load_z(tile + stride);
        f32x16 d2[CT];
        RCX_MLP_ZERO(d2, CT)
        RCX_MLP_STAMP(5)
#pragma unroll 1
        for (int ht = 0; ht < HT; ++ht) {
            hidden_tile_ring<KS1, CT, 4>(Lf + (size_t)ht * NCH * 64, Lb1 + 32 * ht, lane, h, zb, d2 RCX_MLP_STAMP_PASS);
            RCX_MLP_STAMP_STEP
        }
        u32x4q xq[NP];
#pragma unroll
        for (int p = 0; p < NP; ++p) xq[p] = __builtin_bit_cast(u32x4q, __builtin_amdgcn_raw_buffer_load_b128(xsrc, (int)(base + ot * RB + 2u * OC * p + ob), 0, 0));
#pragma unroll
        for (int p = 0; p < NP; ++p) {
#pragma unroll
            for (int g = 2 * (p & 1); g < 2 * (p & 1) + 2; ++g) RCX_MLP_IMAGE_QUAD(d2[p >> 1], Lb2 + 32 * (p >> 1) + 8 * g + 4 * h, Lt + r * OP + 4 * (8 * (g & 1) + 4 * h))
            wave_sync();
            const unsigned char* src = Lt + ot * OP + 2 * ob;
            const f32x4q lo = *reinterpret_cast<const f32x4q*>(src), hi = *reinterpret_cast<const f32x4q*>(src + 16);
            __builtin_amdgcn_raw_buffer_store_b128(__builtin_bit_cast(u32x4q, rows_plus_x(lo, hi, xq[p])), ysrc, (int)(base + ot * RB + 2u * OC * p + ob), 0, 0);
            wave_sync();
        }
    }
    RCX_MLP_STAMP(5)
    RCX_MLP_STAMP_END(wv * (int)gridDim.x + (int)blockIdx.x)
}


template <int KS1, int HT, int CT, int RD, int NW = 8>
__global__ void __launch_bounds__(64 * NW, 2)
k_channel_mlp_wide(const bf16_t* __restrict__ z, const bf16_t* __restrict__ xres, bf16_t* __restrict__ y, const u32x4q* __restrict__ wfrag, const float* __restrict__ bias, int M)
{
    extern __shared__ __attribute__((aligned(16))) unsigned char lds_raw[];
    constexpr int NT = 64 * NW, SH = NW, NST = HT / SH, NCH = KS1 + 2 * CT, NF = KS1 + 4 * SH;
    static_assert(CT == 2 * NW && NW <= 8 && HT % SH == 0 && NF % RD == 0 && KS1 % RD == 0 && KS1 % 8 == 0, "a hidden tile (phase A) and two output tiles (phase B) per wave");
    constexpr int XP = NST & 1;
    constexpr int ZR = KS1 / 4, ZU = 8 * ZR / NW;
    static_assert(8 * ZR % NW == 0, "the z requests divide among the waves");
    using L = WideLds<KS1, HT, CT, NW>;
    constexpr int RB = 32 * KS1, OP = L::OP, XBYTES = L::XBYTES;
    u32x4q* const Lz = reinterpret_cast<u32x4q*>(lds_raw);
    u32x4q* const Lx = reinterpret_cast<u32x4q*>(lds_raw + L::xchg);
    float* const Lb1 = reinterpret_cast<float*>(lds_raw + L::b1);
    const float* const Lb2 = Lb1 + 32 * HT;
    const int lane = threadIdx.x & 63, r = lane & 31, h = lane >> 5;
    const int wv = __builtin_amdgcn_readfirstlane(threadIdx.x >> 6);
    auto frag = [&](int s, int i) -> u32x4q {
        const int ht = SH * s + (i < KS1 ? wv : (i - KS1) >> 2);
        const int f = i < KS1 ? i : KS1 + 4 * wv + 2 * ((i - KS1) & 1) + (((i - KS1) >> 1) & 1);
        return wfrag[((size_t)ht * NCH + f) * 64 + lane];
    };
    u32x4q ring[RD];
#pragma unroll
    for (int i = 0; i < RD; ++i) ring[i] = frag(0, i);
    const unsigned nbytes = (unsigned)M * (unsigned)RB;
    const __amdgpu_buffer_rsrc_t zsrc = token_rows(z, nbytes), xsrc = token_rows(xres, nbytes), ysrc = token_rows(y, nbytes);
    const unsigned base = blockIdx.x * 64u * RB;
    {
        u32x4q zq[ZU];
#pragma unroll
        for (int i = 0; i < ZU; ++i) {
            const int tg = ZU == ZR ? wv : (ZU * wv + i) / ZR, j = ZU == ZR ? i : (ZU * wv + i) % ZR;
            zq[i] = __builtin_bit_cast(u32x4q, __builtin_amdgcn_raw_buffer_load_b128(zsrc, (int)(base + (8u * tg + (lane & 7)) * RB + 16u * (lane >> 3) + 128u * j), 0, 0));
        }
        for (int i = threadIdx.x; i < 32 * (HT + CT); i += NT) Lb1[i] = bias[i];
#pragma unroll
        for (int i = 0; i < ZU; ++i) {
            const int tg = ZU == ZR ? wv : (ZU * wv + i) / ZR, j = ZU == ZR ? i : (ZU * wv + i) % ZR;
            Lz[((tg >> 2) * KS1 + (lane >> 4) + 4 * j) * 64 + ((lane >> 3) & 1) * 32 + 8 * (tg & 3) + (lane & 7)] = zq[i];
        }
    }
    __syncthreads();
    if (!(__builtin_popcount(wv) & 1)) __builtin_amdgcn_s_setprio(1);
    constexpr int LGKM0 = 0xC07F;
    f32x16 d2[2][2];
    RCX_MLP_ZERO(d2[0], 2)
    RCX_MLP_ZERO(d2[1], 2)
    const unsigned ot = lane >> 3, ob = 16u * (lane & 7);
    u32x4q xq[2][4];
    auto step = [&](int s, auto last_c) {
        constexpr bool LAST = decltype(last_c)::value;
        const int sn = LAST ? 0 : s + 1;
        f32x16 d1[2];
        RCX_MLP_ZERO(d1, 2)
        constexpr int BD = 2;
        u32x4q zb[BD][2];
#pragma unroll
        for (int k = 0; k < BD; ++k)
#pragma unroll
            for (int tt = 0; tt < 2; ++tt) zb[k][tt] = Lz[(tt * KS1 + k) * 64 + lane];
#pragma unroll
        for (int ks = 0; ks < KS1; ++ks) {
            const bf16x8 a = __builtin_bit_cast(bf16x8, ring[ks % RD]);
            ring[ks % RD] = frag(s, ks + RD);
            const bf16x8 b0 = __builtin_bit_cast(bf16x8, zb[ks % BD][0]), b1 = __builtin_bit_cast(bf16x8, zb[ks % BD][1]);
            if (ks + BD < KS1) {
#pragma unroll
                for (int tt = 0; tt < 2; ++tt) zb[ks % BD][tt] = Lz[(tt * KS1 + ks + BD) * 64 + lane];
            }
            d1[0] = __builtin_amdgcn_mfma_f32_32x32x16_bf16(a, b0, d1[0], 0, 0, 0);
            d1[1] = __builtin_amdgcn_mfma_f32_32x32x16_bf16(a, b1, d1[1], 0, 0, 0);
            __builtin_amdgcn_sched_barrier(0);
        }
        const float* const b1t = Lb1 + 32 * (SH * s + wv);
        u32x4q* const Lw = Lx + (size_t)((s + XP) & 1) * (XBYTES / 16) + wv * 4 * 64 + lane;
#pragma unroll
        for (int tt = 0; tt < 2; ++tt) {
            RCX_MLP_HIDDEN_GELU(d1[tt], *reinterpret_cast<const f32x4q*>(b1t + 8 * g + 4 * h))
            Lw[(2 * tt) * 64] = __builtin_bit_cast(u32x4q, hb[0]);
            Lw[(2 * tt + 1) * 64] = __builtin_bit_cast(u32x4q, hb[1]);
        }
        __builtin_amdgcn_s_waitcnt(LGKM0);
        __builtin_amdgcn_s_barrier();
        if constexpr (LAST) {
#pragma unroll
            for (int tt = 0; tt < 2; ++tt)
#pragma unroll
                for (int j = 0; j < 4; ++j)
                    xq[tt][j] = __builtin_bit_cast(u32x4q, __builtin_amdgcn_raw_buffer_load_b128(xsrc, (int)(base + (32u * tt + 8u * j + ot) * RB + 128u * wv + ob), 0, 0));
        }
        const u32x4q* const Lr = Lx + (size_t)((s + XP) & 1) * (XBYTES / 16) + lane;
        u32x4q hq[2][2][2];
#pragma unroll
        for (int tt = 0; tt < 2; ++tt)
#pragma unroll
            for (int q = 0; q < 2; ++q) hq[0][tt][q] = Lr[(2 * tt + q) * 64];
#pragma unroll
        for (int hl = 0; hl < SH; ++hl) {
            if (hl + 1 < SH) {
#pragma unroll
                for (int tt = 0; tt < 2; ++tt)
#pragma unroll
                    for (int q = 0; q < 2; ++q) hq[(hl + 1) & 1][tt][q] = Lr[((hl + 1) * 4 + 2 * tt + q) * 64];
            }
#pragma unroll
            for (int j = 0; j < 4; ++j) {
                const int i = KS1 + 4 * hl + j, c2 = j & 1, q = j >> 1;
                const bf16x8 a = __builtin_bit_cast(bf16x8, ring[i % RD]);
                if (i + RD < NF) ring[i % RD] = frag(s, i + RD);
                else if (!LAST) ring[i % RD] = frag(sn, i + RD - NF);
                d2[c2][0] = __builtin_amdgcn_mfma_f32_32x32x16_bf16(a, __builtin_bit_cast(bf16x8, hq[hl & 1][0][q]), d2[c2][0], 0, 0, 0);
                d2[c2][1] = __builtin_amdgcn_mfma_f32_32x32x16_bf16(a, __builtin_bit_cast(bf16x8, hq[hl & 1][1][q]), d2[c2][1], 0, 0, 0);
                __builtin_amdgcn_sched_barrier(0);
            }
        }
    };
#pragma unroll 1
    for (int s = 0; s < NST - 1; ++s) step(s, std::false_type{});
    step(NST - 1, std::true_type{});
    unsigned char* const Lt = lds_raw + (size_t)wv * L::IMG;
#pragma unroll
    for (int tt = 0; tt < 2; ++tt) {
#pragma unroll
        for (int c2 = 0; c2 < 2; ++c2)
#pragma unroll
            for (int g = 0; g < 4; ++g) RCX_MLP_IMAGE_QUAD(d2[c2][tt], Lb2 + 32 * (2 * wv + c2) + 8 * g + 4 * h, Lt + r * OP + 4 * (32 * c2 + 8 * g + 4 * h))
        wave_sync();
#pragma unroll
        for (int j = 0; j < 4; ++j) {
            const unsigned char* src = Lt + (8 * j + ot) * OP + 2 * ob;
            const f32x4q lo = *reinterpret_cast<const f32x4q*>(src), hi = *reinterpret_cast<const f32x4q*>(src + 16);
            __builtin_amdgcn_raw_buffer_store_b128(__builtin_bit_cast(u32x4q, rows_plus_x(lo, hi, xq[tt][j])), ysrc, (int)(base + (32u * tt + 8u * j + ot) * RB + 128u * wv + ob), 0, 0);
        }
        wave_sync();
    }
}

}

constexpr int mlp_ks1(int C) { return (C + 15) / 16; }
constexpr int mlp_ct(int C) { return C > 128 ? (C + 63) / 64 * 2 : (C + 31) / 32; }

static bool mlp_shape(int C, int H, int* ks1, int* ht, int* ct)
{
    if (C <= 0 || H <= 0 || C % 8 || H % 32) return false;
    *ks1 = mlp_ks1(C); *ht = H / 32; *ct = mlp_ct(C);
    return true;
}

size_t channel_mlp_pack_bytes(int C, int H)
{
    int ks1, ht, ct;
    if (!mlp_shape(C, H, &ks1, &ht, &ct)) return 0;
    return (size_t)(ht * ks1 + ct * 2 * ht) * 1024;
}

#define RCX_MLP_LAUNCH_ARGS const void* z, const void* x, void* y, const void* wfrag, const float* bias, int M, int C, int ncu, hipStream_t s
typedef hipError_t (*mlp_launcher)(RCX_MLP_LAUNCH_ARGS);

template <int CH, int HT>
static hipError_t launch_mlp(RCX_MLP_LAUNCH_ARGS)
{
    constexpr int KS1 = mlp_ks1(CH), CT = mlp_ct(CH);
    constexpr int NW = CT <= 2 ? 12 : 8, WPS = NW / 4;
    constexpr bool STAGED = CT <= 2;
    using L = mlp::SmallLds<KS1, HT, CT, NW, STAGED>;
    static_assert(L::bytes <= 160 * 1024, "weights + the waves' images must fit the LDS");
    if (C != CH) return hipErrorInvalidConfiguration;
    auto kfn = mlp::k_channel_mlp<KS1, HT, CT, NW, WPS, CH == 16 * KS1, CH == 32 * CT, STAGED>;
    RCX_SET_LDS_ONCE(kfn, L::bytes);
    const int ntiles = (M + 31) / 32;
    int grid = ncu;
    if (grid * NW > ntiles) grid = (ntiles + NW - 1) / NW;
    hipLaunchKernelGGL(kfn, dim3((unsigned)grid), dim3(64 * NW), L::bytes, s, (const bf16_t*)z, (const bf16_t*)x, (bf16_t*)y, (const mlp::u32x4q*)wfrag, bias, M, C, ntiles RCX_MLP_STAMP_VAL);
    return hipGetLastError();
}

template <int CH, int HT, int ZH = 1, bool ZPF = true>
static hipError_t launch_mlp_stream(RCX_MLP_LAUNCH_ARGS)
{
    constexpr int KS1 = mlp_ks1(CH), CT = mlp_ct(CH), NW = 4;
    using L = mlp::StreamLds<KS1, HT, CT, NW, ZH>;
    static_assert(L::bytes <= 160 * 1024, "the ring and the waves' images must fit the LDS");
    static_assert(CH == 16 * KS1, "no padding lanes");
    if (C != CH) return hipErrorInvalidConfiguration;
    auto kfn = mlp::k_channel_mlp_stream<KS1, HT, CT, NW, NW / 4, ZH, ZPF>;
    RCX_SET_LDS_ONCE(kfn, L::bytes);
    const int nblocks = (M + 32 * NW - 1) / (32 * NW);
    const int grid = nblocks < ncu ? nblocks : ncu;
    hipLaunchKernelGGL(kfn, dim3((unsigned)grid), dim3(64 * NW), L::bytes, s, (const bf16_t*)z, (const bf16_t*)x, (bf16_t*)y, (const mlp::u32x4q*)wfrag, bias, M, C, nblocks);
    return hipGetLastError();
}

template <int CH, int HT>
static hipError_t launch_mlp_pair(RCX_MLP_LAUNCH_ARGS)
{
    constexpr int KS1 = mlp_ks1(CH), CT = mlp_ct(CH);
    using L = mlp::PairLds<KS1, HT, CT>;
    static_assert(L::bytes <= 160 * 1024, "the ring and the waves' images must fit the LDS");
    static_assert(CH == 16 * KS1, "no padding lanes");
    if (C != CH) return hipErrorInvalidConfiguration;
    auto kfn = mlp::k_channel_mlp_pair<KS1, HT, CT, RCX_MLP_PINNED>;
    RCX_SET_LDS_ONCE(kfn, L::bytes);
    const int nblocks = (M + 32 * L::NW - 1) / (32 * L::NW);
    const int grid = nblocks < ncu ? nblocks : ncu;
    hipLaunchKernelGGL(kfn, dim3((unsigned)grid), dim3(64 * L::NW), L::bytes, s, (const bf16_t*)z, (const bf16_t*)x, (bf16_t*)y, (const mlp::u32x4q*)wfrag, bias, M, C, nblocks RCX_MLP_STAMP_VAL);
    return hipGetLastError();
}

template <int CH, int HT>
static hipError_t launch_mlp_res128(RCX_MLP_LAUNCH_ARGS)
{
    constexpr int KS1 = mlp_ks1(CH), CT = mlp_ct(CH);
    using L = mlp::Res128Lds<KS1, HT, CT>;
    static_assert(L::bytes <= 160 * 1024, "the pack, the biases and the waves' images must fit the LDS");
    static_assert(CH == 16 * KS1, "no padding lanes");
    if (C != CH) return hipErrorInvalidConfiguration;
    auto kfn = mlp::k_channel_mlp_res128<KS1, HT, CT>;
    RCX_SET_LDS_ONCE(kfn, L::bytes);
    const int ntiles = (M + 31) / 32;
    int grid = (ntiles + L::NW - 1) / L::NW;
    if (grid > ncu) grid = ncu;
    hipLaunchKernelGGL(kfn, dim3((unsigned)grid), dim3(64 * L::NW), L::bytes, s, (const bf16_t*)z, (const bf16_t*)x, (bf16_t*)y, (const mlp::u32x4q*)wfrag, bias, M, ntiles RCX_MLP_STAMP_VAL);
    return hipGetLastError();
}

template <int CH, int HT>
static hipError_t launch_mlp_wide(RCX_MLP_LAUNCH_ARGS)
{
    constexpr int KS1 = mlp_ks1(CH), CT = mlp_ct(CH), NW = CT / 2;
    using L = mlp::WideLds<KS1, HT, CT, NW>;
    static_assert(L::bytes <= 160 * 1024, "the z fragments, the exchange buffers and the biases must fit the LDS");
    static_assert(CH == 16 * KS1, "no padding lanes");
    if (C != CH) return hipErrorInvalidConfiguration;
    auto kfn = mlp::k_channel_mlp_wide<KS1, HT, CT, 8, NW>;
    RCX_SET_LDS_ONCE(kfn, L::bytes);
    hipLaunchKernelGGL(kfn, dim3((unsigned)((M + 63) / 64)), dim3(64 * NW), L::bytes, s, (const bf16_t*)z, (const bf16_t*)x, (bf16_t*)y, (const mlp::u32x4q*)wfrag, bias, M);
    return hipGetLastError();
}

struct MlpRow { int C, HT, min_tokens; mlp_launcher launch; };
static constexpr MlpRow MLP_ROWS[] = {
    {256, 16, 1, launch_mlp_pair<256, 16>},
    {128, 8, 1, launch_mlp_res128<128, 8>},
    {512, 32, 2048, launch_mlp_wide<512, 32>},
    {512, 24, 512, launch_mlp_wide<512, 24>},
    {384, 24, 784, launch_mlp_wide<384, 24>},
    {192, 12, 1, launch_mlp_stream<192, 12>},
    {160, 10, 1, launch_mlp_stream<160, 10>},
    {320, 20, 1, launch_mlp_stream<320, 20, 2, false>},
    {64, 4, 1, launch_mlp<64, 4>},
    {56, 4, 1, launch_mlp<56, 4>},
    {48, 3, 1, launch_mlp<48, 3>},
    {40, 3, 1, launch_mlp<40, 3>},
    {96, 6, 1, launch_mlp<96, 6>},
    {80, 5, 1, launch_mlp<80, 5>},
};

static const MlpRow* mlp_row(int M, int C, int H, int dtype)
{
    if (dtype != 1 || M <= 0 || H <= 0 || H % 32) return nullptr;
    if ((unsigned long long)M * C * 2 >= (1ull << 31)) return nullptr;
    for (const MlpRow& row : MLP_ROWS)
        if (row.C == C && row.HT == H / 32) return M >= row.min_tokens ? &row : nullptr;
    return nullptr;
}

bool channel_mlp_applicable(int M, int C, int H, int dtype) { return mlp_row(M, C, H, dtype) != nullptr; }

hipError_t channel_mlp(const void* z, const void* x, void* y, const void* wfrag, const float* bias, int M, int C, int H, int dtype, hipStream_t s)
{
    const MlpRow* const row = mlp_row(M, C, H, dtype);
    if (!row) return hipErrorInvalidConfiguration;
    static std::atomic<int> cus[RCX_MAX_DEVICES];
    int dev = 0, ncu = 256;
    if (hipGetDevice(&dev) == hipSuccess && dev >= 0 && dev < RCX_MAX_DEVICES) {
        ncu = cus[dev].load(std::memory_order_relaxed);
        if (ncu <= 0) {
            int v = 0;
            ncu = hipDeviceGetAttribute(&v, hipDeviceAttributeMultiprocessorCount, dev) == hipSuccess && v > 0 ? v : 256;
            cus[dev].store(ncu, std::memory_order_relaxed);
        }
    }
    return row->launch(z, x, y, wfrag, bias, M, C, ncu, s);
}

}

#ifdef RCX_MLP_STAMPS
extern "C" int rcx_mlp_diag_fwd(const void* z, const void* x, void* y, const void* wfrag, const float* bias, int M, int C, int H, void* stamps, void* stream)
{
    rcx::g_stamps = (unsigned long long*)stamps;
    return (int)rcx::channel_mlp(z, x, y, wfrag, bias, M, C, H, 1, (hipStream_t)stream);
}
#endif
```

recnext_amd/csrc/rcx_opts.h:

```cpp
#pragma once
#include <stdlib.h>
#include <mutex>
#include <string>

namespace rcx {
namespace opt {

enum Id { FORCE_GENERIC, CPL, CPL14, CPL14_RL, CPT, CPT_CB, CPT16, UPADD_CPL, UPADD_CPT, NESTED, TRAIN_FUSED, BWD_FUSED, WGRAD_CPL, COUNT };

namespace detail {
inline const char* name_of(int i)
{
    static const char* const k[COUNT] = {"RCX_FORCE_GENERIC", "RCX_CPL", "RCX_CPL14", "RCX_CPL14_RL", "RCX_CPT", "RCX_CPT_CB", "RCX_CPT16",
                                         "RCX_UPADD_CPL", "RCX_UPADD_CPT", "RCX_NESTED", "RCX_TRAIN_FUSED", "RCX_BWD_FUSED", "RCX_WGRAD_CPL"};
    return k[i];
}
struct Table {
    std::string val[COUNT];
    std::once_flag once;
    void read()
    {
        for (int i = 0; i < COUNT; ++i) {
            const char* v = getenv(name_of(i));
            val[i] = v ? v : "";
        }
    }
};
inline Table& table() { static Table t; return t; }
}

inline const char* str(Id id)
{
    detail::Table& t = detail::table();
    std::call_once(t.once, [&] { t.read(); });
    return t.val[id].c_str();
}
inline bool off(Id id) { return str(id)[0] == '0'; }
inline bool on(Id id) { const char* v = str(id); return *v && *v != '0'; }
inline int int_or(Id id, int dflt) { const char* v = str(id); return *v ? atoi(v) : dflt; }
inline void reload()
{
    detail::Table& t = detail::table();
    std::call_once(t.once, [&] { t.read(); });
    t.read();
}

inline bool hand_kernels_off() { return on(FORCE_GENERIC); }

}
}
```

recnext_amd/layers.py:

```python
import torch
import torch.nn as nn


def _bn_affine(norm):
    scale = norm.weight / torch.sqrt(norm.running_var + norm.eps)
    return scale, norm.bias - scale * norm.running_mean


class ConvNorm(nn.Sequential):
    def __init__(self, in_channels, out_channels, kernel_size=1, stride=1, padding=0, dilation=1, groups=1,
                 bias=False, bn_weight_init=1):
        super().__init__()
        self.add_module("conv", nn.Conv2d(in_channels, out_channels, kernel_size, stride, padding, dilation, groups, bias=bias))
        self.add_module("norm", nn.BatchNorm2d(out_channels))
        nn.init.constant_(self.norm.weight, bn_weight_init)
        nn.init.constant_(self.norm.bias, 0)

    @torch.no_grad()
    def fuse(self):
        conv = self.conv
        scale, shift = _bn_affine(self.norm)
        if conv.bias is not None:
            shift = shift + scale * conv.bias
        out = nn.Conv2d(conv.in_channels, conv.out_channels, conv.kernel_size, stride=conv.stride, padding=conv.padding,
                        dilation=conv.dilation, groups=conv.groups, bias=True, device=conv.weight.device,
                        dtype=conv.weight.dtype)
        out.weight.copy_(conv.weight * scale.view(-1, 1, 1, 1))
        out.bias.copy_(shift)
        return out


class NormLinear(nn.Sequential):
    def __init__(self, in_channels, out_channels, bias=True, std=0.02):
        super().__init__()
        self.add_module("norm", nn.BatchNorm1d(in_channels))
        self.add_module("linear", nn.Linear(in_channels, out_channels, bias=bias))
        nn.init.trunc_normal_(self.linear.weight, std=std)
        if bias:
            nn.init.constant_(self.linear.bias, 0)

    @torch.no_grad()
    def fuse(self):
        lin = self.linear
        scale, shift = _bn_affine(self.norm)
        out = nn.Linear(lin.in_features, lin.out_features, bias=True, device=lin.weight.device, dtype=lin.weight.dtype)
        out.weight.copy_(lin.weight * scale.view(1, -1))
        b = lin.weight @ shift
        out.bias.copy_(b if lin.bias is None else b + lin.bias)
        return out


class DropPath(nn.Module):

    def __init__(self, drop_prob=0.0):
        super().__init__()
        self.drop_prob = drop_prob

    def forward(self, x):
        if not self.training or self.drop_prob == 0.0:
            return x
        keep = 1.0 - self.drop_prob
        mask = x.new_empty((x.shape[0],) + (1,) * (x.dim() - 1)).bernoulli_(keep)
        return x * mask.div_(keep)


class PointwiseLinear(nn.Module):

    def __init__(self, conv):
        super().__init__()
        if conv.kernel_size != (1, 1) or conv.groups != 1 or conv.stride != (1, 1) or conv.padding != (0, 0):
            raise ValueError("PointwiseLinear replaces a dense 1x1, stride-1 convolution")
        self.weight, self.bias = conv.weight, conv.bias
        self.in_channels, self.out_channels = conv.in_channels, conv.out_channels
        self.out_padded, self.in_padded = self.out_channels, self.in_channels
        self._pad_key, self._pad_w, self._pad_b = None, None, None

    def pad(self, out_to=None, in_to=None):
        out_to = self.out_channels if out_to is None else int(out_to)
        in_to = self.in_channels if in_to is None else int(in_to)
        if out_to < self.out_channels or in_to < self.in_channels:
            raise ValueError("padding cannot shrink a layer")
        self.out_padded, self.in_padded, self._pad_key = out_to, in_to, None
        return self

    def _operands(self):
        w, b = self.weight, self.bias
        if self.out_padded == self.out_channels and self.in_padded == self.in_channels:
            return w.view(self.out_channels, self.in_channels), b
        key = (w.data_ptr(), w._version, w.dtype, w.device, None if b is None else (b.data_ptr(), b._version))
        if key != self._pad_key:
            with torch.no_grad():
                wp = w.new_zeros(self.out_padded, self.in_padded)
                wp[:self.out_channels, :self.in_channels] = w.view(self.out_channels, self.in_channels)
                bp = None
                if b is not None:
                    bp = b.new_zeros(self.out_padded)
                    bp[:self.out_channels] = b
            self._pad_key, self._pad_w, self._pad_b = key, wp, bp
        return self._pad_w, self._pad_b

    def forward(self, x):
        n, c, h, w = x.shape
        if c != self.in_padded:
            raise ValueError(f"expected {self.in_padded} input channels, got {c}")
        wt, b = self._operands()
        x2 = x.permute(0, 2, 3, 1)
        y2 = torch.nn.functional.linear(x2.reshape(n * h * w, c), wt, b)
        return y2.view(n, h, w, self.out_padded).permute(0, 3, 1, 2)


def _is_exact_gelu(m):
    return type(m) is nn.GELU and getattr(m, "approximate", "none") == "none"


def _needs_grad(*tensors):
    return torch.is_grad_enabled() and any(t is not None and t.requires_grad for t in tensors)


class FusedChannelMlp:

    def __init__(self, fc1, fc2):
        self.fc1, self.fc2 = fc1, fc2
        self._key, self._pack = None, None

    def supported(self, x):
        from . import ops
        n, c, h, w = x.shape
        return x.is_cuda and x.dtype == torch.bfloat16 and ops.channel_mlp_hidden(n * h * w, c, self.fc1.out_channels, x.dtype) > 0

    def usable(self, seq, t, x):
        if len(seq) != 3 or seq[0] is not self.fc1 or seq[2] is not self.fc2 or not _is_exact_gelu(seq[1]):
            return False
        if t.dtype != x.dtype or t.device != x.device or self.fc1.weight.device != x.device or self.fc2.weight.device != x.device:
            return False
        if _needs_grad(t, x, self.fc1.weight, self.fc1.bias, self.fc2.weight, self.fc2.bias):
            return False
        return self.supported(x)

    def packs(self):
        return [] if self._pack is None else [p for p in self._pack if torch.is_tensor(p)]

    def _operands(self, hidden_to):
        from . import ops
        ts = [self.fc1.weight, self.fc1.bias, self.fc2.weight, self.fc2.bias]
        key = (hidden_to,) + tuple(None if t is None else (t.data_ptr(), t._version, t.dtype, t.device) for t in ts)
        if key != self._key:
            self._pack = ops.pack_channel_mlp(*ts, hidden_to=hidden_to)
            self._key = key
        return self._pack

    def __call__(self, z, x):
        from . import ops
        n, c, h, w = x.shape
        wfrag, bias, hidden = self._operands(ops.channel_mlp_hidden(n * h * w, c, self.fc1.out_channels, x.dtype))
        return ops.channel_mlp(z, x, wfrag, bias, hidden)


class FusedStem:

    def __init__(self, conv1, conv2):
        self.conv1, self.conv2 = conv1, conv2
        self._key, self._pack = None, None

    def supported(self, x):
        from . import ops
        n, c, h, w = x.shape
        return x.is_cuda and x.dtype == torch.bfloat16 and c == 3 and ops.stem_supported(n, h, w, self.conv1.out_channels, self.conv2.out_channels, x.dtype)

    def usable(self, seq, x):
        if len(seq) != 3 or seq[0] is not self.conv1 or seq[2] is not self.conv2 or not _is_exact_gelu(seq[1]):
            return False
        if self.conv1.weight.device != x.device or self.conv2.weight.device != x.device:
            return False
        if _needs_grad(x, self.conv1.weight, self.conv1.bias, self.conv2.weight, self.conv2.bias):
            return False
        return self.supported(x)

    def packs(self):
        return [] if self._pack is None else [p for p in self._pack if torch.is_tensor(p)]

    def __call__(self, x):
        from . import ops
        ts = [self.conv1.weight, self.conv1.bias, self.conv2.weight, self.conv2.bias]
        key = tuple(None if t is None else (t.data_ptr(), t._version, t.dtype, t.device) for t in ts)
        if key != self._key:
            self._pack = ops.pack_stem(*ts)
            self._key = key
        return ops.stem(x, *self._pack, self.conv1.out_channels, self.conv2.out_channels)


class FusedStem3:

    def __init__(self, conv1, conv2, conv3, final_act):
        self.convs, self.final_act = (conv1, conv2, conv3), bool(final_act)
        self._key, self._pack = None, None

    def _params(self):
        return [t for c in self.convs for t in (c.weight, c.bias)]

    def supported(self, x):
        from . import ops
        n, c, h, w = x.shape
        c1, c2, c3 = (m.out_channels for m in self.convs)
        return x.is_cuda and x.dtype == torch.bfloat16 and c == 3 and (4 * c1, 2 * c2) == (c3, c3) and ops.stem3_supported(n, h, w, c3, self.final_act, x.dtype)

    def usable(self, seq, x):
        if len(seq) != 6 or any(seq[2 * i] is not m for i, m in enumerate(self.convs)) or not _is_exact_gelu(seq[1]) or not _is_exact_gelu(seq[3]):
            return False
        if not (_is_exact_gelu(seq[5]) if self.final_act else type(seq[5]) is nn.Identity):
            return False
        if any(m.weight.device != x.device for m in self.convs) or _needs_grad(x, *self._params()):
            return False
        return x.dim() == 4 and x.is_contiguous(memory_format=torch.channels_last) and self.supported(x)

    def packs(self):
        return [] if self._pack is None else [p for p in self._pack if torch.is_tensor(p)]

    def __call__(self, x):
        from . import ops
        ts = self._params()
        key = tuple(None if t is None else (t.data_ptr(), t._version, t.dtype, t.device) for t in ts)
        if key != self._key:
            self._pack = ops.pack_stem3(*ts)
            self._key = key
        return ops.stem3(x, *self._pack, self.convs[2].out_channels, self.final_act)
```

recnext_amd/models.py:

```python
import torch
import torch.nn as nn

from .layers import ConvNorm, DropPath, NormLinear
from .recattn import RecAttn2d
from .recconv import RecConv2d

CONFIGS = {
    "recnext_m0": dict(family="m", embed_dim=(40, 80, 160, 320), depth=(2, 2, 9, 1)),
    "recnext_m1": dict(family="m", embed_dim=(48, 96, 192, 384), depth=(3, 3, 15, 2)),
    "recnext_m2": dict(family="m", embed_dim=(56, 112, 224, 448), depth=(3, 3, 15, 2)),
    "recnext_m3": dict(family="m", embed_dim=(64, 128, 256, 512), depth=(3, 3, 13, 2)),
    "recnext_m4": dict(family="m", embed_dim=(64, 128, 256, 512), depth=(5, 5, 25, 4), drop_path=0.2),
    "recnext_m5": dict(family="m", embed_dim=(80, 160, 320, 640), depth=(7, 7, 35, 2), drop_path=0.3),
    "recnext_a0": dict(family="a", embed_dim=(40, 80, 160, 320), depth=(2, 2, 9, 1)),
    "recnext_a1": dict(family="a", embed_dim=(48, 96, 192, 384), depth=(3, 3, 15, 2)),
    "recnext_a2": dict(family="a", embed_dim=(56, 112, 224, 448), depth=(3, 3, 15, 2)),
    "recnext_a3": dict(family="a", embed_dim=(64, 128, 256, 512), depth=(3, 3, 13, 2), mlp_ratio=1.875),
    "recnext_a4": dict(family="a", embed_dim=(64, 128, 256, 512), depth=(5, 5, 25, 4), mlp_ratio=1.875, drop_path=0.2),
    "recnext_a5": dict(family="a", embed_dim=(80, 160, 320, 640), depth=(7, 7, 35, 2), mlp_ratio=1.875, drop_path=0.3),
}


def default_token_mixer(family):
    if family == "m":
        return lambda dim, stage: RecConv2d(dim, level=4 - stage, kernel_size=5)
    if family == "a":
        return lambda dim, stage: RecAttn2d(dim, num_heads=2 ** (stage + 1), stage=stage)
    raise ValueError(f"unknown family {family!r}")


def channel_mlp(dim, hidden, act_layer):
    return nn.Sequential(ConvNorm(dim, int(hidden), kernel_size=1), act_layer(), ConvNorm(int(hidden), dim, kernel_size=1))


class RecNextStem(nn.Module):
    def __init__(self, in_channels, out_channels, act_layer=nn.GELU):
        super().__init__()
        self.stem = nn.Sequential(ConvNorm(in_channels, out_channels // 2, kernel_size=3, stride=2, padding=1), act_layer(),
                                  ConvNorm(out_channels // 2, out_channels, kernel_size=3, stride=2, padding=1))

    def forward(self, x):
        fused = self.__dict__.get("_fused_stem")
        if fused is not None and not self.training and fused.usable(self.stem, x):
            return fused(x)
        return self.stem(x)


class MetaNeXtBlock(nn.Module):

    def __init__(self, dim, mlp_ratio, act_layer, stage, drop_path, family, token_mixer):
        super().__init__()
        self.token_mixer = token_mixer(dim, stage)
        if family == "m":
            self.norm = nn.BatchNorm2d(dim)
        self.channel_mixer = channel_mlp(dim, dim * mlp_ratio, act_layer)
        self.drop_path = DropPath(drop_path) if drop_path > 0.0 else nn.Identity()
        self._has_norm = family == "m"

    def forward(self, x):
        t = self.token_mixer(x)
        if self._has_norm:
            t = self.norm(t)
        fused = self.__dict__.get("_fused_mlp")
        if fused is not None and not self.training and fused.usable(self.channel_mixer, t, x):
            return fused(t, x)
        return x + self.drop_path(self.channel_mixer(t))


class Downsample(nn.Module):
    def __init__(self, in_channels, mlp_ratio, act_layer):
        super().__init__()
        out_channels = in_channels * 2
        self.token_mixer = nn.Conv2d(in_channels, out_channels, kernel_size=7, padding=3, groups=in_channels, stride=2)
        self.norm = nn.BatchNorm2d(out_channels)
        self.channel_mixer = channel_mlp(out_channels, out_channels * mlp_ratio, act_layer)
        object.__setattr__(self, "_hip", None)

    def _hip_path(self):
        hip = self.__dict__.get("_hip")
        if hip is not None and (hip.token_mixer is not self.token_mixer or hip.norm is not self.norm):
            hip = None
            if isinstance(self.token_mixer, nn.Conv2d) and type(self.norm) is nn.BatchNorm2d:
                from .dwconv import DownsampleDwConv
                try:
                    hip = DownsampleDwConv(self.token_mixer, self.norm)
                except ValueError:
                    hip = None
            object.__setattr__(self, "_hip", hip)
        return hip

    def forward(self, x):
        hip = self._hip_path()
        x = hip(x) if hip is not None else self.norm(self.token_mixer(x))
        fused = self.__dict__.get("_fused_mlp")
        if fused is not None and not self.training and fused.usable(self.channel_mixer, x, x):
            return fused(x, x)
        return x + self.channel_mixer(x)


class RecNextClassifier(nn.Module):
    def __init__(self, dim, num_classes, distillation=False, drop=0.0):
        super().__init__()
        self.head_drop = nn.Dropout(drop)
        self.head = NormLinear(dim, num_classes) if num_classes > 0 else nn.Identity()
        self.head_dist = NormLinear(dim, num_classes) if num_classes > 0 else nn.Identity()
        self.distillation = distillation
        self.num_classes = num_classes

    def forward(self, x):
        x = self.head_drop(x)
        a, b = self.head(x), self.head_dist(x)
        if self.training and self.distillation:
            return a, b
        return (a + b) / 2

    @torch.no_grad()
    def fuse(self):
        if self.num_classes <= 0:
            return nn.Identity()
        a, b = self.head.fuse(), self.head_dist.fuse()
        a.weight.copy_((a.weight + b.weight) / 2)
        a.bias.copy_((a.bias + b.bias) / 2)
        return a


class RecNextStage(nn.Module):
    def __init__(self, in_channels, out_channels, depth, mlp_ratio, act_layer, downsample, stage, drop_path, family, token_mixer):
        super().__init__()
        self.downsample = Downsample(in_channels, mlp_ratio, act_layer) if downsample else nn.Identity()
        self.blocks = nn.Sequential(*[MetaNeXtBlock(out_channels, mlp_ratio, act_layer, stage, drop_path, family, token_mixer)
                                      for _ in range(depth)])

    def forward(self, x):
        return self.blocks(self.downsample(x))


class RecNext(nn.Module):
    def __init__(self, family="m", in_chans=3, embed_dim=(48,), depth=(2,), mlp_ratio=2, global_pool="avg", num_classes=1000,
                 act_layer=nn.GELU, distillation=False, drop_rate=0.0, drop_path=0.0, token_mixer=None):
        super().__init__()
        token_mixer = token_mixer or default_token_mixer(family)
        self.family = family
        self.global_pool = global_pool
        self.embed_dim = tuple(embed_dim)
        self.num_classes = num_classes
        self.stem = RecNextStem(in_chans, embed_dim[0], act_layer)
        stages, prev = [], embed_dim[0]
        for i, (dim, d) in enumerate(zip(embed_dim, depth)):
            stages.append(RecNextStage(prev, dim, d, mlp_ratio, act_layer, downsample=i != 0, stage=i, drop_path=drop_path,
                                       family=family, token_mixer=token_mixer))
            prev = dim
        self.stages = nn.Sequential(*stages)
        self.num_features = embed_dim[-1]
        self.head_drop = nn.Dropout(drop_rate)
        self.head = RecNextClassifier(embed_dim[-1], num_classes, distillation)

    def forward_features(self, x):
        return self.stages(self.stem(x))

    def forward_head(self, x):
        if self.global_pool == "avg":
            x = x.mean((2, 3))
        return self.head(self.head_drop(x))

    def forward(self, x):
        return self.forward_head(self.forward_features(x))


def create_model(name, distillation=False, token_mixer=None, **overrides):
    if name not in CONFIGS:
        from . import lsmodels
        if name in lsmodels.LS_CONFIGS:
            return lsmodels.create_model(name, distillation=distillation, token_mixer=token_mixer, **overrides)
        from . import lsshare
        if name in lsshare.SHARE_CONFIGS:
            return lsshare.create_model(name, distillation=distillation, token_mixer=token_mixer, **overrides)
    cfg = dict(CONFIGS[name])
    if distillation:
        cfg["drop_path"] = 0.0
    cfg.update(overrides)
    return RecNext(distillation=distillation, token_mixer=token_mixer, **cfg)


def _mlp_hosts():
    from . import lsmodels
    return (MetaNeXtBlock, Downsample, lsmodels.MetaNeXtBlock, lsmodels.Downsample)


def replace_batchnorm(net):
    for name, child in list(net.named_children()):
        if hasattr(child, "fuse"):
            fused = child.fuse()
            setattr(net, name, fused)
            replace_batchnorm(fused)
        else:
            replace_batchnorm(child)
    return net


@torch.no_grad()
def fold_token_mixer_norms(net):
    n = 0
    for m in net.modules():
        if isinstance(m, MetaNeXtBlock) and m._has_norm and isinstance(m.norm, nn.BatchNorm2d) \
                and isinstance(m.token_mixer, RecConv2d):
            if m.norm.training:
                raise RuntimeError("fold_token_mixer_norms needs eval mode (running statistics)")
            bn = m.norm
            scale = bn.weight.float() / torch.sqrt(bn.running_var.float() + bn.eps)
            shift = bn.bias.float() - scale * bn.running_mean.float()
            m.token_mixer.fold_output_affine(scale, shift)
            m.norm = nn.Identity()
            m._has_norm = False
            n += 1
    return n


@torch.no_grad()
def use_hip_downsample(net):
    from . import lsmodels
    from .dwconv import DownsampleDwConv
    n = 0
    for m in net.modules():
        if isinstance(m, Downsample) and m._hip is None and isinstance(m.token_mixer, nn.Conv2d) and isinstance(m.norm, nn.BatchNorm2d):
            object.__setattr__(m, "_hip", DownsampleDwConv(m.token_mixer, m.norm))
            n += 1
        elif isinstance(m, lsmodels.Downsample) and not m.__dict__.get("_hip") and m._conv() is not None:
            m._hip = True
            n += 1
    return n


def use_hip_batchnorm(net, all_shapes=False):
    from .batchnorm import HipBatchNorm2d
    n = 0
    for m in net.modules():
        if type(m) is nn.BatchNorm2d:
            m.__class__ = HipBatchNorm2d
            if all_shapes:
                m.hip_all_shapes = True
            n += 1
    return n


def use_fused_rep_train(net, all_shapes=False):
    from . import lsmodels
    n = 0
    for m in net.modules():
        if isinstance(m, lsmodels.RepVGGDW):
            n += 0 if m.__dict__.get("_fused_rep_train") else 1
            m._fused_rep_train = "all" if all_shapes else "measured"
    return n


def use_linear_pointwise(net):
    from .layers import PointwiseLinear
    n = 0
    for m in net.modules():
        if isinstance(m, _mlp_hosts()):
            seq = m.channel_mixer
            for i, sub in enumerate(seq):
                if isinstance(sub, nn.Conv2d) and sub.kernel_size == (1, 1) and sub.groups == 1 and sub.bias is not None:
                    seq[i] = PointwiseLinear(sub)
                    n += 1
    return n


def use_fused_stem(net):
    from .layers import FusedStem, FusedStem3, _is_exact_gelu
    from .lsmodels import RecNextStem as LsStem

    def stem_conv(m):
        return isinstance(m, nn.Conv2d) and m.kernel_size == (3, 3) and m.stride == (2, 2) and m.padding == (1, 1) and m.groups == 1 and m.dilation == (1, 1)

    n = 0
    for m in net.modules():
        if not isinstance(m, (RecNextStem, LsStem)) or m.__dict__.get("_fused_stem") is not None:
            continue
        seq = m.stem
        if isinstance(m, RecNextStem):
            if len(seq) == 3 and stem_conv(seq[0]) and stem_conv(seq[2]) and _is_exact_gelu(seq[1]) and seq[0].in_channels == 3:
                object.__setattr__(m, "_fused_stem", FusedStem(seq[0], seq[2]))
                n += 1
        elif len(seq) == 6 and all(stem_conv(seq[i]) and seq[i].bias is not None for i in (0, 2, 4)) and _is_exact_gelu(seq[1]) and _is_exact_gelu(seq[3]) \
                and (_is_exact_gelu(seq[5]) or type(seq[5]) is nn.Identity) and seq[0].in_channels == 3:
            object.__setattr__(m, "_fused_stem", FusedStem3(seq[0], seq[2], seq[4], _is_exact_gelu(seq[5])))
            n += 1
    return n


def use_fused_mlp(net):
    from .layers import FusedChannelMlp, PointwiseLinear
    n = 0
    for m in net.modules():
        if isinstance(m, _mlp_hosts()) and m.__dict__.get("_fused_mlp") is None:
            seq = m.channel_mixer
            if len(seq) == 3 and isinstance(seq[0], PointwiseLinear) and isinstance(seq[2], PointwiseLinear) and isinstance(seq[1], nn.GELU) \
                    and getattr(seq[1], "approximate", "none") == "none":
                object.__setattr__(m, "_fused_mlp", FusedChannelMlp(seq[0], seq[2]))
                n += 1
    return n


def padded_hidden_width(hidden, max_growth=0.125):
    for mult in (64, 16):
        hp = -(-hidden // mult) * mult
        if hp != hidden and hp <= hidden * (1 + max_growth):
            return hp
    return hidden


def pad_mlp_hidden(net):
    from .layers import PointwiseLinear
    n = 0
    for m in net.modules():
        if isinstance(m, _mlp_hosts()):
            seq = m.channel_mixer
            if len(seq) != 3 or not isinstance(seq[0], PointwiseLinear) or not isinstance(seq[2], PointwiseLinear):
                continue
            with torch.no_grad():
                if float(seq[1](torch.zeros(1)).abs().max()) != 0.0:
                    continue
            hp = padded_hidden_width(seq[0].out_channels)
            if hp != seq[0].out_padded or hp != seq[2].in_padded:
                seq[0].pad(out_to=hp)
                seq[2].pad(in_to=hp)
                n += hp != seq[0].out_channels
    return n


def token_mixer_shapes(name, resolution=224):
    cfg = CONFIGS[name]
    out = []
    side = resolution // 4
    for s, (dim, d) in enumerate(zip(cfg["embed_dim"], cfg["depth"])):
        out.append((dim, side, side, 4 - s if cfg["family"] == "m" else None, d))
        side = (side + 1) // 2 if s < 3 else side
    return out


def token_mixer_algorithmic_bytes(name, resolution=224, elem_bytes=2, k=5):
    total = 0
    for (c, h, w, level, count) in token_mixer_shapes(name, resolution):
        if level is None:
            raise ValueError("defined for the M family")
        total += count * (2 * c * h * w * elem_bytes + (level + 2) * c * k * k * elem_bytes)
    return total
```

recnext_amd/ops.py:

```python
import torch

from . import _lib

_DT = {torch.float32: _lib.DTYPE_F32, torch.bfloat16: _lib.DTYPE_BF16, torch.float16: _lib.DTYPE_F16}


_D16_CHECKED = set()


def selftest_d16(device):
    dev = torch.device(device)
    src = (torch.arange(64, device=dev, dtype=torch.int32) * 517 + 0x1234).to(torch.int16)
    flag = torch.zeros(1, dtype=torch.int32, device=dev)
    with torch.cuda.device(dev):
        rc = _lib.load().rcx_selftest_d16(src.data_ptr(), flag.data_ptr(), _stream(dev))
    _lib.check(rc, "rcx_selftest_d16")
    mask = int(flag.item())
    if mask:
        raise _lib.RcxError(f"D16 self-test failed on {dev} (mask {mask:#x}: bit 0 global_load_short_d16_hi, 1 buffer_load_short_d16_hi, 2 "
                            "ds_read_u16_d16_hi): this device does not zero the other half of a D16-hi load; the 16-bit kernels would return garbage")
    _D16_CHECKED.add(dev.index if dev.index is not None else torch.cuda.current_device())
    return mask


# ... 470 lines not shown
        raise ValueError(f"ls_recattn: no kernel for a {h} x {w} plane, C={c}, split={split}, {heads} heads, {x.dtype} (ls_recattn_supported)")
    x = _nhwc(x, "x")
    r = torch.empty_like(x, memory_format=torch.channels_last)
    t = torch.empty_like(x, memory_format=torch.channels_last)
    with _on(x.device):
        rc = _lib.load().rcx_ls_recattn_fwd(x.data_ptr(), r.data_ptr(), t.data_ptr(), w_rep.data_ptr(), b_rep.data_ptr(), w_down_kkc.data_ptr(), b_down.data_ptr(),
                                            wqT.data_ptr(), bq.data_ptr(), wkT.data_ptr(), bk.data_ptr(), w_pe_kkc.data_ptr(), b_pe.data_ptr(),
                                            w_conv_kkc.data_ptr(), b_conv.data_ptr(), b, h, w, c, split, heads, _dt(x), _stream(x.device))
    _lib.check(rc, "rcx_ls_recattn_fwd")
    return r, t


def ls_la3(x, w_rep, b_rep, wqT, bq, wkT, bk, w_pe_kkc, b_pe, split, heads):
    c = x.shape[1] if torch.is_tensor(x) and x.dim() == 4 else 0
    _check_ls_args("ls_la3", x, split, [("w_rep", w_rep, 9 * c), ("b_rep", b_rep, c), ("wqT", wqT, split * (split // 2)), ("bq", bq, split // 2),
                                        ("wkT", wkT, split * (split // 2)), ("bk", bk, split // 2), ("w_pe_kkc", w_pe_kkc, 9 * split), ("b_pe", b_pe, split)])
    b, _, h, w = x.shape
    if not ls_la3_supported(b, h, w, c, split, heads, x.dtype):
        raise ValueError(f"ls_la3: no kernel for a {h} x {w} plane, C={c}, split={split}, {heads} heads, {x.dtype} (ls_la3_supported)")
    x = _nhwc(x, "x")
    r = torch.empty_like(x, memory_format=torch.channels_last)
    t = torch.empty_like(x, memory_format=torch.channels_last)
    with _on(x.device):
        rc = _lib.load().rcx_ls_la3_fwd(x.data_ptr(), r.data_ptr(), t.data_ptr(), w_rep.data_ptr(), b_rep.data_ptr(), wqT.data_ptr(), bq.data_ptr(),
                                        wkT.data_ptr(), bk.data_ptr(), w_pe_kkc.data_ptr(), b_pe.data_ptr(), b, h, w, c, split, heads, _dt(x), _stream(x.device))
    _lib.check(rc, "rcx_ls_la3_fwd")
    return r, t


def ls_recattn_tiled_supported(b, h, w, c, split, heads, dtype):
    return dtype in _DT and _lib.load().rcx_ls_recattn_tiled_supported(b, h, w, c, split, heads, _DT[dtype]) > 0


def ls_la3_tiled_supported(b, h, w, c, split, heads, dtype):
    return dtype in _DT and _lib.load().rcx_ls_la3_tiled_supported(b, h, w, c, split, heads, _DT[dtype]) > 0


def _ls_workspace(x, nbytes, workspace):
    if workspace is None:
        return torch.empty(nbytes // 4, dtype=torch.float32, device=x.device)
    if not torch.is_tensor(workspace) or workspace.dtype != torch.float32 or workspace.device != x.device or not workspace.is_contiguous():
        raise ValueError("workspace must be a contiguous float32 tensor on x's device")
    if workspace.numel() * 4 < nbytes:
        raise ValueError(f"workspace of {workspace.numel() * 4} bytes, {nbytes} needed")
    return workspace


def ls_recattn_tiled(x, w_rep, b_rep, w_down_kkc, b_down, wqT, bq, wkT, bk, w_pe_kkc, b_pe, w_conv_kkc, b_conv, split, heads=1, workspace=None):
    c = x.shape[1] if torch.is_tensor(x) and x.dim() == 4 else 0
    _check_ls_args("ls_recattn_tiled", x, split, [("w_rep", w_rep, 9 * c), ("b_rep", b_rep, c), ("w_down_kkc", w_down_kkc, 25 * split), ("b_down", b_down, split),
                                                  ("wqT", wqT, split * (split // 2)), ("bq", bq, split), ("wkT", wkT, split * (split // 2)), ("bk", bk, split),
                                                  ("w_pe_kkc", w_pe_kkc, 9 * split), ("b_pe", b_pe, split), ("w_conv_kkc", w_conv_kkc, 25 * split), ("b_conv", b_conv, split)])
    b, _, h, w = x.shape
    if not ls_recattn_tiled_supported(b, h, w, c, split, heads, x.dtype):
        raise ValueError(f"ls_recattn_tiled: no kernel for a {h} x {w} plane, C={c}, split={split}, {heads} heads, {x.dtype} (ls_recattn_tiled_supported)")
    lib = _lib.load()
    nbytes = lib.rcx_ls_recattn_tiled_workspace_bytes(b, h, w, c, split, heads, _dt(x))
    x = _nhwc(x, "x")
    with _on(x.device):
        ws = _ls_workspace(x, nbytes, workspace)
        r = torch.empty_like(x, memory_format=torch.channels_last)
        t = torch.empty_like(x, memory_format=torch.channels_last)
        rc = lib.rcx_ls_recattn_tiled_fwd(x.data_ptr(), r.data_ptr(), t.data_ptr(), w_rep.data_ptr(), b_rep.data_ptr(), w_down_kkc.data_ptr(), b_down.data_ptr(),
                                          wqT.data_ptr(), bq.data_ptr(), wkT.data_ptr(), bk.data_ptr(), w_pe_kkc.data_ptr(), b_pe.data_ptr(),
                                          w_conv_kkc.data_ptr(), b_conv.data_ptr(), ws.data_ptr(), ws.numel() * 4, b, h, w, c, split, heads, _dt(x),
                                          _stream(x.device))
    _lib.check(rc, "rcx_ls_recattn_tiled_fwd")
    return r, t


def ls_la3_tiled(x, w_rep, b_rep, wqT, bq, wkT, bk, w_pe_kkc, b_pe, split, heads, workspace=None):
    c = x.shape[1] if torch.is_tensor(x) and x.dim() == 4 else 0
    _check_ls_args("ls_la3_tiled", x, split, [("w_rep", w_rep, 9 * c), ("b_rep", b_rep, c), ("wqT", wqT, split * (split // 2)), ("bq", bq, split // 2),
                                              ("wkT", wkT, split * (split // 2)), ("bk", bk, split // 2), ("w_pe_kkc", w_pe_kkc, 9 * split), ("b_pe", b_pe, split)])
    b, _, h, w = x.shape
    if not ls_la3_tiled_supported(b, h, w, c, split, heads, x.dtype):
        raise ValueError(f"ls_la3_tiled: no kernel for a {h} x {w} plane, C={c}, split={split}, {heads} heads, {x.dtype} (ls_la3_tiled_supported)")
    lib = _lib.load()
    nbytes = lib.rcx_ls_la3_tiled_workspace_bytes(b, h, w, c, split, heads, _dt(x))
    x = _nhwc(x, "x")
    with _on(x.device):
        ws = _ls_workspace(x, nbytes, workspace)
        r = torch.empty_like(x, memory_format=torch.channels_last)
        t = torch.empty_like(x, memory_format=torch.channels_last)
        rc = lib.rcx_ls_la3_tiled_fwd(x.data_ptr(), r.data_ptr(), t.data_ptr(), w_rep.data_ptr(), b_rep.data_ptr(), wqT.data_ptr(), bq.data_ptr(),
                                      wkT.data_ptr(), bk.data_ptr(), w_pe_kkc.data_ptr(), b_pe.data_ptr(), ws.data_ptr(), ws.numel() * 4,
                                      b, h, w, c, split, heads, _dt(x), _stream(x.device))
    _lib.check(rc, "rcx_ls_la3_tiled_fwd")
    return r, t


def _mlp_acc_unit(i, h):
    return (i & 3) + 8 * (i >> 2) + 4 * h


def channel_mlp_hidden(m, c, hidden, dtype):
    if dtype != torch.bfloat16:
        return 0
    lib = _lib.load()
    for mult in (32, 64, 128):
        hp = -(-int(hidden) // mult) * mult
        if hp <= 1.125 * hidden + 31 and lib.rcx_channel_mlp_supported(int(m), int(c), hp, _DT[dtype]) > 0:
            return hp
    return 0


def channel_mlp_supported(m, c, hidden, dtype):
    return channel_mlp_hidden(m, c, hidden, dtype) > 0


def _mlp_tiles(c, hidden):
    ks1, ht, ct = -(-c // 16), hidden // 32, -(-c // 32)
    if c > 128 and ct % 2:
        ct += 1
    return ks1, ht, ct


def pack_channel_mlp(w1, b1, w2, b2, hidden_to=None):
    w1 = w1.detach().reshape(w1.shape[0], -1)
    w2 = w2.detach().reshape(w2.shape[0], -1)
    h0, c = w1.shape
    if tuple(w2.shape) != (c, h0):
        raise ValueError(f"w2 must be ({c}, {h0}), got {tuple(w2.shape)}")
    dev = w1.device
    hp = -(-h0 // 32) * 32 if hidden_to is None else int(hidden_to)
    if hp % 32 or hp < h0:
        raise ValueError(f"hidden_to={hidden_to} must be a multiple of 32 and at least {h0}")
    ks1, ht, ct = _mlp_tiles(c, hp)
    w1p = torch.zeros(32 * ht, 16 * ks1, dtype=torch.bfloat16, device=dev)
    w1p[:h0, :c] = w1.to(torch.bfloat16)
    f1 = w1p.view(ht, 32, ks1, 2, 8).permute(0, 2, 3, 1, 4)
    w2p = torch.zeros(32 * ct, 32 * ht, dtype=torch.bfloat16, device=dev)
    w2p[:c, :h0] = (0.5 * w2.float()).to(torch.bfloat16)
    unit = torch.tensor([[[_mlp_acc_unit(8 * q + j, h) for j in range(8)] for h in range(2)] for q in range(2)], device=dev)
    f2 = w2p.view(ct, 32, ht, 32)[:, :, :, unit]
    f2 = f2.permute(0, 2, 3, 4, 1, 5)
    f1 = f1.reshape(ht, ks1 * 512)
    f2 = f2.reshape(ct, ht, 2, 512).permute(1, 0, 2, 3).reshape(ht, ct * 2 * 512)
    wfrag = torch.cat([f1, f2], dim=1).reshape(-1).contiguous()
    bias = torch.zeros(32 * (ht + ct), dtype=torch.float32, device=dev)
    if b1 is not None:
        bias[:h0] = b1.detach().float()
    if b2 is not None:
        bias[32 * ht:32 * ht + c] = b2.detach().float()
    return wfrag, bias, 32 * ht


def _check_pack(t, dtype, numel, device, name):
    if not torch.is_tensor(t) or t.dtype != dtype or t.numel() != numel or not t.is_contiguous() or t.device != device:
        got = f"{tuple(t.shape)} {t.dtype} on {t.device}" if torch.is_tensor(t) else type(t).__name__
        raise ValueError(f"{name} must be a contiguous {dtype} tensor of {numel} elements on {device}, got {got}")


def channel_mlp(z, x, wfrag, bias, hidden):
    z = _nhwc(z, "z")
    x = _nhwc(x, "x")
    if z.shape != x.shape or z.dtype != x.dtype:
        raise ValueError("z and x must have the same shape and dtype")
    n, c, h, w = x.shape
    lib = _lib.load()
    if wfrag.dtype != torch.bfloat16 or wfrag.numel() * 2 != lib.rcx_channel_mlp_pack_bytes(c, hidden) or not wfrag.is_contiguous():
        raise ValueError("wfrag is not the pack of pack_channel_mlp for this (C, H)")
    _check_pack(bias, torch.float32, hidden + 32 * _mlp_tiles(c, hidden)[2], x.device, "bias")
    _check_pack(wfrag, torch.bfloat16, wfrag.numel(), x.device, "wfrag")
    if z.device != x.device:
        raise ValueError("z and x must be on the same device")
    y = _empty_nhwc(n, c, h, w, x.dtype, x.device)
    with _on(x.device):
        rc = lib.rcx_channel_mlp_fwd(z.data_ptr(), x.data_ptr(), y.data_ptr(), wfrag.data_ptr(), bias.data_ptr(), n * h * w, c, hidden, _dt(x), _stream(x.device))
    _lib.check(rc, "rcx_channel_mlp_fwd")
    return y


def stem_supported(n, h, w, cm, co, dtype):
    return dtype == torch.bfloat16 and _lib.load().rcx_stem_supported(int(n), int(h), int(w), int(cm), int(co), _DT[dtype]) > 0


def _pack_conv3x3_frags(w, b):
    co, ci = w.shape[0], w.shape[1]
    dev = w.device
    kc, mt = -(-ci // 16) * 16, -(-co // 32)
    wp = torch.zeros(32 * mt, kc, 9, dtype=torch.bfloat16, device=dev)
    wp[:co, :ci] = w.detach().reshape(co, ci, 9).to(torch.bfloat16)
    f = wp.view(mt, 32, kc // 16, 2, 8, 9).permute(0, 5, 2, 3, 1, 4)
    bp = torch.zeros(32 * mt, dtype=torch.float32, device=dev)
    if b is not None:
        bp[:co] = b.detach().float()
    return f.reshape(-1).contiguous(), bp


def pack_stem(w1, b1, w2, b2):
    cm, co = w1.shape[0], w2.shape[0]
    if tuple(w1.shape) != (cm, 3, 3, 3) or tuple(w2.shape) != (co, cm, 3, 3):
        raise ValueError(f"stem weights must be (CM, 3, 3, 3) and (CO, CM, 3, 3), got {tuple(w1.shape)} and {tuple(w2.shape)}")
    dev = w1.device
    m1 = -(-cm // 32)
    w1k = torch.zeros(32 * m1, 32, dtype=torch.bfloat16, device=dev)
    w1k[:cm, :27] = w1.detach().permute(0, 2, 3, 1).reshape(cm, 27).to(torch.bfloat16)
    w1p = w1k.view(m1, 32, 2, 2, 8).permute(0, 2, 3, 1, 4).reshape(-1).contiguous()
    b1p = torch.zeros(32 * m1, dtype=torch.float32, device=dev)
    if b1 is not None:
        b1p[:cm] = b1.detach().float()
    w2frag, b2p = _pack_conv3x3_frags(w2, b2)
    return w1p, b1p, w2frag, b2p


def stem(x, w1p, b1p, w2frag, b2p, cm, co):
    x = _nhwc(x, "x")
    n, c, h, w = x.shape
    if c != 3:
        raise ValueError(f"the stem takes 3 input channels, got {c}")
    h2, w2_ = -(-(-(-h // 2)) // 2), -(-(-(-w // 2)) // 2)
    m1, mt = -(-cm // 32), -(-co // 32)
    _check_pack(w1p, torch.bfloat16, m1 * 2 * 512, x.device, "w1p")
    _check_pack(b1p, torch.float32, 32 * m1, x.device, "b1p")
    _check_pack(w2frag, torch.bfloat16, _lib.load().rcx_stem_pack_bytes(cm, co) // 2, x.device, "w2frag")
    _check_pack(b2p, torch.float32, 32 * mt, x.device, "b2p")
    y = _empty_nhwc(n, co, h2, w2_, x.dtype, x.device)
    with _on(x.device):
        rc = _lib.load().rcx_stem_fwd(x.data_ptr(), y.data_ptr(), w1p.data_ptr(), b1p.data_ptr(), w2frag.data_ptr(), b2p.data_ptr(), n, h, w, cm, co, _dt(x), _stream(x.device))
    _lib.check(rc, "rcx_stem_fwd")
    return y


def linear_attention_core_backward(qpre, kpre, v, gout, heads):
    v = _nhwc(v, "v")
    gout = _nhwc(gout, "grad_output")
    b, c, h, w = v.shape
    n = h * w
    if gout.dtype != v.dtype:
        gout = gout.to(v.dtype)
    gq = torch.empty_like(qpre)
    gk = torch.empty_like(kpre)
    gv = _empty_nhwc(b, c, h, w, v.dtype, v.device)
    with _on(v.device):
        rc = _lib.load().rcx_linear_attention_bwd(qpre.data_ptr(), kpre.data_ptr(), v.data_ptr(), gout.data_ptr(),
                                                  gq.data_ptr(), gk.data_ptr(), gv.data_ptr(), b, n, c, heads, _dt(v), _stream(v.device))
    _lib.check(rc, "rcx_linear_attention_bwd")
    return gq, gk, gv


class LinearAttentionCoreFn(torch.autograd.Function):

    @staticmethod
    def forward(ctx, qpre, kpre, v, pe, heads):
        out = linear_attention_core(qpre, kpre, v, pe, heads)
        ctx.save_for_backward(qpre, kpre, v)
        ctx.heads = heads
        return out

    @staticmethod
    def backward(ctx, gout):
        qpre, kpre, v = ctx.saved_tensors
        gq, gk, gv = linear_attention_core_backward(qpre, kpre, v, gout, ctx.heads)
        return gq, gk, gv, gout, None


def linear_attention_wide_supported(b, n, cqk, cv, heads, dtype):
    code = _DT.get(dtype)
    return code is not None and _lib.load().rcx_linear_attention_wide_supported(b, n, cqk, cv, heads, code) == 1


def _check_wide_args(fn, qpre, kpre, v, other, other_name, heads):
    for name, t in (("qpre", qpre), ("kpre", kpre), ("v", v), (other_name, other)):
        if not isinstance(t, torch.Tensor):
            raise ValueError(f"{fn}: {name} must be a tensor, got {type(t).__name__}")
    for name, t in (("qpre", qpre), ("kpre", kpre), ("v", v), (other_name, other)):
        if not t.is_cuda:
            raise ValueError(f"{fn}: {name} is on {t.device}: the wide linear-attention core runs on the GPU only (HIP kernels)")
        if t.device != v.device:
            raise ValueError(f"{fn}: {name} is on {t.device}, v on {v.device}")
    if v.dim() != 4:
        raise ValueError(f"{fn}: v must be 4-D (N, Cv, h, w), got shape {tuple(v.shape)}")
    if v.dtype not in _DT:
        raise ValueError(f"{fn}: v must be float32, bfloat16 or float16, got {v.dtype}")
    b, cv, h, w = v.shape
    n = h * w
    if qpre.dim() != 3 or qpre.shape[0] != b or qpre.shape[1] != n:
        raise ValueError(f"{fn}: qpre must be ({b}, {n}, Cqk), got {tuple(qpre.shape)}")
    cqk = qpre.shape[2]
    for name, t in (("qpre", qpre), ("kpre", kpre)):
        if tuple(t.shape) != (b, n, cqk) or not t.is_contiguous() or t.dtype != v.dtype:
            raise ValueError(f"{fn}: {name} must be a contiguous ({b}, {n}, {cqk}) tensor of {v.dtype}, got {tuple(t.shape)} {t.dtype}")
    if tuple(other.shape) != tuple(v.shape):
        raise ValueError(f"{fn}: {other_name} has shape {tuple(other.shape)}, expected v's {tuple(v.shape)}")
    if other_name == "pe" and other.dtype != v.dtype:
        raise ValueError(f"{fn}: pe must have v's dtype {v.dtype}, got {other.dtype}")
    if not isinstance(heads, int) or heads <= 0 or cqk % heads or cv % heads:
        raise ValueError(f"{fn}: heads={heads} must be a positive integer dividing Cqk={cqk} and Cv={cv}")
    if not linear_attention_wide_supported(b, n, cqk, cv, heads, v.dtype):
        raise ValueError(f"{fn}: no kernel for heads of {cqk // heads} (q / k) x {cv // heads} (v) channels: both must be multiples of 4 from 4 to 128")
    return b, n, cqk, cv, h, w


def linear_attention_wide(qpre, kpre, v, pe, heads):
    b, n, cqk, cv, h, w = _check_wide_args("linear_attention_wide", qpre, kpre, v, pe, "pe", heads)
    v = _nhwc(v, "v")
    pe = _nhwc(pe, "pe")
    out = _empty_nhwc(b, cv, h, w, v.dtype, v.device)
    with _on(v.device):
        rc = _lib.load().rcx_linear_attention_wide_fwd(qpre.data_ptr(), kpre.data_ptr(), v.data_ptr(), pe.data_ptr(), out.data_ptr(),
                                                       b, n, cqk, cv, heads, _dt(v), _stream(v.device))
    _lib.check(rc, "rcx_linear_attention_wide_fwd")
    return out


def linear_attention_wide_backward(qpre, kpre, v, gout, heads):
    b, n, cqk, cv, h, w = _check_wide_args("linear_attention_wide_backward", qpre, kpre, v, gout, "grad_output", heads)
    v = _nhwc(v, "v")
    gout = _nhwc(gout, "grad_output")
    if gout.dtype != v.dtype:
        gout = gout.to(v.dtype)
    gq = torch.empty_like(qpre)
    gk = torch.empty_like(kpre)
    gv = _empty_nhwc(b, cv, h, w, v.dtype, v.device)
    with _on(v.device):
        rc = _lib.load().rcx_linear_attention_wide_bwd(qpre.data_ptr(), kpre.data_ptr(), v.data_ptr(), gout.data_ptr(),
                                                       gq.data_ptr(), gk.data_ptr(), gv.data_ptr(), b, n, cqk, cv, heads, _dt(v), _stream(v.device))
    _lib.check(rc, "rcx_linear_attention_wide_bwd")
    return gq, gk, gv


class LinearAttentionWideCoreFn(torch.autograd.Function):

# ... 102 lines not shown
```

Measured before the change: 119,000.

## Fuse global average pool into last channel MLP and software-pipeline GELU with MFMA

```diff
diff --git a/include/recnext_amd.h b/include/recnext_amd.h
--- a/include/recnext_amd.h
+++ b/include/recnext_amd.h
@@ -109,6 +109,8 @@
 int rcx_channel_mlp_supported(int M, int C, int H, int dtype);
 size_t rcx_channel_mlp_pack_bytes(int C, int H);
 int rcx_channel_mlp_fwd(const void* z, const void* x, void* y, const void* wfrag, const float* bias, int M, int C, int H, int dtype, void* stream);
+int rcx_channel_mlp_pool_supported(int N, int P, int C, int H, int dtype);
+int rcx_channel_mlp_pool_fwd(const void* z, const void* x, void* y, void* pooled, const void* wfrag, const float* bias, int N, int P, int C, int H, int dtype, void* stream);
 
 int rcx_stem_supported(int N, int H, int W, int CM, int CO, int dtype);
 size_t rcx_stem_pack_bytes(int CM, int CO);
diff --git a/recnext_amd/_lib.py b/recnext_amd/_lib.py
--- a/recnext_amd/_lib.py
+++ b/recnext_amd/_lib.py
@@ -60,6 +60,8 @@
     "rcx_channel_mlp_supported": (_i, [_i] * 4),
     "rcx_channel_mlp_pack_bytes": (_sz, [_i] * 2),
     "rcx_channel_mlp_fwd": (_i, [_vp] * 5 + [_i] * 4 + [_vp]),
+    "rcx_channel_mlp_pool_supported": (_i, [_i] * 5),
+    "rcx_channel_mlp_pool_fwd": (_i, [_vp] * 6 + [_i] * 5 + [_vp]),
     "rcx_recattn2d_fwd_supported": (_i, [_i] * 7),
     "rcx_recattn2d_fwd": (_i, [_vp] * 10 + [_i] * 7 + [_vp]),
     "rcx_dwconv2d_bwd_workspace_bytes": (ctypes.c_size_t, [_i, _i]),
diff --git a/recnext_amd/csrc/rcx_api.hip b/recnext_amd/csrc/rcx_api.hip
--- a/recnext_amd/csrc/rcx_api.hip
+++ b/recnext_amd/csrc/rcx_api.hip
@@ -1105,6 +1105,23 @@
     return e == hipSuccess ? 0 : hip_fail(e, "rcx_channel_mlp_fwd");
 }
 
+int rcx_channel_mlp_pool_supported(int N, int P, int C, int H, int dtype) { return rcx::channel_mlp_pool_applicable(N, P, C, H, dtype) ? 1 : 0; }
+
+int rcx_channel_mlp_pool_fwd(const void* z, const void* x, void* y, void* pooled, const void* wfrag, const float* bias, int N, int P, int C, int H, int dtype, void* stream)
+{
+    if (!z || !x || !y || !pooled || !wfrag || !bias) return fail(RCX_ERR_BAD_ARG, "rcx_channel_mlp_pool_fwd: null pointer");
+    if (N <= 0 || P <= 0 || C <= 0 || H <= 0) return fail(RCX_ERR_BAD_ARG, "non-positive extent N=%d P=%d C=%d H=%d", N, P, C, H);
+    if (!known_dtype(dtype)) return fail(RCX_ERR_BAD_ARG, "unknown dtype %d", dtype);
+    if (((size_t)z & 15) || ((size_t)x & 15) || ((size_t)y & 15) || ((size_t)wfrag & 15) || ((size_t)bias & 15) || ((size_t)pooled & 1))
+        return fail(RCX_ERR_BAD_ARG, "rcx_channel_mlp_pool_fwd: z, x, y, wfrag and bias must be 16-byte aligned, pooled 2-byte aligned");
+    if (y == z || y == x || pooled == z || pooled == x || pooled == y) return fail(RCX_ERR_BAD_ARG, "rcx_channel_mlp_pool_fwd: y and pooled must alias neither an input nor each other");
+    if (!rcx::channel_mlp_pool_applicable(N, P, C, H, dtype))
+        return fail(RCX_ERR_UNSUPPORTED, "rcx_channel_mlp_pool_fwd: no kernel for N=%d P=%d C=%d H=%d dtype %d (bf16; (C, H) = (384, 768), (512, 768), (512, 1024) from the token count N P "
+                                         "rcx_channel_mlp_supported accepts; P <= 64; RCX_MLP_POOL=0 switches it off)", N, P, C, H, dtype);
+    hipError_t e = rcx::channel_mlp_pool(z, x, y, pooled, wfrag, bias, N, P, C, H, dtype, (hipStream_t)stream);
+    return e == hipSuccess ? 0 : hip_fail(e, "rcx_channel_mlp_pool_fwd");
+}
+
 int rcx_ls_recattn_supported(int B, int H, int W, int C, int split, int heads, int dtype)
 {
     return rcx::ls_recattn_applicable(B, H, W, C, split, heads, dtype) ? 1 : 0;
diff --git a/recnext_amd/csrc/rcx_launch.h b/recnext_amd/csrc/rcx_launch.h
--- a/recnext_amd/csrc/rcx_launch.h
+++ b/recnext_amd/csrc/rcx_launch.h
@@ -148,6 +148,8 @@
 bool channel_mlp_applicable(int M, int C, int H, int dtype);
 size_t channel_mlp_pack_bytes(int C, int H);
 hipError_t channel_mlp(const void* z, const void* x, void* y, const void* wfrag, const float* bias, int M, int C, int H, int dtype, hipStream_t s);
+bool channel_mlp_pool_applicable(int N, int P, int C, int H, int dtype);
+hipError_t channel_mlp_pool(const void* z, const void* x, void* y, void* pooled, const void* wfrag, const float* bias, int N, int P, int C, int H, int dtype, hipStream_t s);
 bool recattn2d_unit_applicable(int B, int H, int W, int C, int heads, int x_dt, int mode);
 hipError_t recattn2d_unit(const void* x, const float* wdn, const float* bdn, const void* wqk_bf16, const float* bqk, const float* wpe, const float* bpe,
                           const float* wcv, const float* bcv, void* y, int B, int H, int C, int heads, int x_dt, hipStream_t s);
diff --git a/recnext_amd/csrc/rcx_mlp.hip b/recnext_amd/csrc/rcx_mlp.hip
--- a/recnext_amd/csrc/rcx_mlp.hip
+++ b/recnext_amd/csrc/rcx_mlp.hip
@@ -1,6 +1,7 @@
 #include "rcx_common.h"
 #include "rcx_launch.h"
 #include "rcx_gelu.h"
+#include "rcx_opts.h"
 #include <type_traits>
 
 #ifdef RCX_MLP_STAMPS
@@ -627,9 +628,10 @@
 }
 
 
-template <int KS1, int HT, int CT, int RD, int NW = 8>
+template <int KS1, int HT, int CT, int RD, int NW = 8, bool POOL = false>
 __global__ void __launch_bounds__(64 * NW, 2)
-k_channel_mlp_wide(const bf16_t* __restrict__ z, const bf16_t* __restrict__ xres, bf16_t* __restrict__ y, const u32x4q* __restrict__ wfrag, const float* __restrict__ bias, int M)
+k_channel_mlp_wide(const bf16_t* __restrict__ z, const bf16_t* __restrict__ xres, bf16_t* __restrict__ y, const u32x4q* __restrict__ wfrag, const float* __restrict__ bias, int M,
+                   bf16_t* __restrict__ pooled, int P RCX_MLP_STAMP_ARG)
 {
     extern __shared__ __attribute__((aligned(16))) unsigned char lds_raw[];
     constexpr int NT = 64 * NW, SH = NW, NST = HT / SH, NCH = KS1 + 2 * CT, NF = KS1 + 4 * SH;
@@ -645,25 +647,31 @@
     const float* const Lb2 = Lb1 + 32 * HT;
     const int lane = threadIdx.x & 63, r = lane & 31, h = lane >> 5;
     const int wv = __builtin_amdgcn_readfirstlane(threadIdx.x >> 6);
-    auto frag = [&](int s, int i) -> u32x4q {
-        const int ht = SH * s + (i < KS1 ? wv : (i - KS1) >> 2);
-        const int f = i < KS1 ? i : KS1 + 4 * wv + 2 * ((i - KS1) & 1) + (((i - KS1) >> 1) & 1);
-        return wfrag[((size_t)ht * NCH + f) * 64 + lane];
-    };
+    auto wf = [&](int ht, int f) -> u32x4q { return wfrag[((size_t)ht * NCH + f) * 64 + lane]; };
+    auto w1f = [&](int s, int ks) -> u32x4q { return wf(SH * s + wv, ks); };
+    auto w2f = [&](int s, int i) -> u32x4q { return wf(SH * s + (i >> 2), KS1 + 4 * wv + 2 * (i & 1) + ((i >> 1) & 1)); };
+    RCX_MLP_STAMP_BEGIN
     u32x4q ring[RD];
 #pragma unroll
-    for (int i = 0; i < RD; ++i) ring[i] = frag(0, i);
-    const unsigned nbytes = (unsigned)M * (unsigned)RB;
-    const __amdgpu_buffer_rsrc_t zsrc = token_rows(z, nbytes), xsrc = token_rows(xres, nbytes), ysrc = token_rows(y, nbytes);
-    const unsigned base = blockIdx.x * 64u * RB;
+    for (int i = 0; i < RD; ++i) ring[i] = w1f(0, i);
+    const unsigned nbytes = (unsigned)(POOL ? P : M) * (unsigned)RB;
+    const size_t img = POOL ? (size_t)blockIdx.x * (size_t)nbytes : 0;
+    const __amdgpu_buffer_rsrc_t zsrc = token_rows((const char*)z + img, nbytes), xsrc = token_rows((const char*)xres + img, nbytes), ysrc = token_rows((char*)y + img, nbytes);
+    const unsigned base = POOL ? 0u : blockIdx.x * 64u * RB;
     {
         u32x4q zq[ZU];
+        constexpr int NB = (32 * (HT + CT) + NT - 1) / NT;
+        float bv[NB];
+#pragma unroll
+        for (int i = 0; i < NB; ++i) bv[i] = (int)threadIdx.x + i * NT < 32 * (HT + CT) ? bias[threadIdx.x + i * NT] : 0.f;
 #pragma unroll
         for (int i = 0; i < ZU; ++i) {
             const int tg = ZU == ZR ? wv : (ZU * wv + i) / ZR, j = ZU == ZR ? i : (ZU * wv + i) % ZR;
             zq[i] = __builtin_bit_cast(u32x4q, __builtin_amdgcn_raw_buffer_load_b128(zsrc, (int)(base + (8u * tg + (lane & 7)) * RB + 16u * (lane >> 3) + 128u * j), 0, 0));
         }
-        for (int i = threadIdx.x; i < 32 * (HT + CT); i += NT) Lb1[i] = bias[i];
+#pragma unroll
+        for (int i = 0; i < NB; ++i)
+            if ((int)threadIdx.x + i * NT < 32 * (HT + CT)) Lb1[threadIdx.x + i * NT] = bv[i];
 #pragma unroll
         for (int i = 0; i < ZU; ++i) {
             const int tg = ZU == ZR ? wv : (ZU * wv + i) / ZR, j = ZU == ZR ? i : (ZU * wv + i) % ZR;
@@ -671,6 +679,7 @@
         }
     }
     __syncthreads();
+    RCX_MLP_STAMP(0)
     if (!(__builtin_popcount(wv) & 1)) __builtin_amdgcn_s_setprio(1);
     constexpr int LGKM0 = 0xC07F;
     f32x16 d2[2][2];
@@ -678,10 +687,10 @@
     RCX_MLP_ZERO(d2[1], 2)
     const unsigned ot = lane >> 3, ob = 16u * (lane & 7);
     u32x4q xq[2][4];
-    auto step = [&](int s, auto last_c) {
-        constexpr bool LAST = decltype(last_c)::value;
-        const int sn = LAST ? 0 : s + 1;
-        f32x16 d1[2];
+    static_assert(NST >= 2 && (4 * SH) % RD == 0, "the first product runs one step ahead; every segment of the fragment stream is whole rings");
+    f32x16 d1[2];
+    auto phase_a = [&](int sa, auto pro_c) {
+        constexpr bool PRO = decltype(pro_c)::value;
         RCX_MLP_ZERO(d1, 2)
         constexpr int BD = 2;
         u32x4q zb[BD][2];
@@ -692,7 +701,8 @@
 #pragma unroll
         for (int ks = 0; ks < KS1; ++ks) {
             const bf16x8 a = __builtin_bit_cast(bf16x8, ring[ks % RD]);
-            ring[ks % RD] = frag(s, ks + RD);
+            if (ks + RD < KS1) ring[ks % RD] = w1f(sa, ks + RD);
+            else ring[ks % RD] = PRO ? w1f(sa + 1, ks + RD - KS1) : w2f(sa - 1, ks + RD - KS1);
             const bf16x8 b0 = __builtin_bit_cast(bf16x8, zb[ks % BD][0]), b1 = __builtin_bit_cast(bf16x8, zb[ks % BD][1]);
             if (ks + BD < KS1) {
 #pragma unroll
@@ -702,22 +712,73 @@
             d1[1] = __builtin_amdgcn_mfma_f32_32x32x16_bf16(a, b1, d1[1], 0, 0, 0);
             __builtin_amdgcn_sched_barrier(0);
         }
-        const float* const b1t = Lb1 + 32 * (SH * s + wv);
-        u32x4q* const Lw = Lx + (size_t)((s + XP) & 1) * (XBYTES / 16) + wv * 4 * 64 + lane;
-#pragma unroll
-        for (int tt = 0; tt < 2; ++tt) {
-            RCX_MLP_HIDDEN_GELU(d1[tt], *reinterpret_cast<const f32x4q*>(b1t + 8 * g + 4 * h))
-            Lw[(2 * tt) * 64] = __builtin_bit_cast(u32x4q, hb[0]);
-            Lw[(2 * tt + 1) * 64] = __builtin_bit_cast(u32x4q, hb[1]);
-        }
-        __builtin_amdgcn_s_waitcnt(LGKM0);
-        __builtin_amdgcn_s_barrier();
+    };
+    constexpr int GM = 32;
+    gelu_f32x2 gv[4], gc[4], gs[4], gq[4];
+    f32x4q bq[2];
+    u32x4q hbv;
+    auto gelu_b1 = [&](int sg, int b) {
+        const float* const b1t = Lb1 + 32 * (SH * sg + wv);
+#pragma unroll
+        for (int g2 = 0; g2 < 2; ++g2) bq[g2] = *reinterpret_cast<const f32x4q*>(b1t + 8 * (2 * b + g2) + 4 * h);
+    };
+    auto gelu_piece = [&](int sg, int m) {
+        constexpr float A = 3.95979f;
+        constexpr float C[8] = {7.975682616e-01f, -1.320175529e-01f, 1.908149943e-02f, -2.016084734e-03f, 1.481452055e-04f, -7.052111414e-06f, 1.927494679e-07f, -2.273170097e-09f};
+        const int tt = m >> 4, b = (m >> 3) & 1, st = m & 7;
+        if (st == 0) {
+#pragma unroll
+            for (int g2 = 0; g2 < 2; ++g2) {
+                const int g = 2 * b + g2;
+                gv[2 * g2] = gelu_f32x2{d1[tt][4 * g] + bq[g2].x, d1[tt][4 * g + 1] + bq[g2].y};
+                gv[2 * g2 + 1] = gelu_f32x2{d1[tt][4 * g + 2] + bq[g2].z, d1[tt][4 * g + 3] + bq[g2].w};
+            }
+#pragma unroll
+            for (int i = 0; i < 2; ++i) gc[i] = gelu_f32x2{__builtin_amdgcn_fmed3f(gv[i].x, -A, A), __builtin_amdgcn_fmed3f(gv[i].y, -A, A)};
+        } else if (st == 1) {
+#pragma unroll
+            for (int i = 2; i < 4; ++i) gc[i] = gelu_f32x2{__builtin_amdgcn_fmed3f(gv[i].x, -A, A), __builtin_amdgcn_fmed3f(gv[i].y, -A, A)};
+#pragma unroll
+            for (int i = 0; i < 4; ++i) gs[i] = gc[i] * gc[i];
+        } else if (st == 2) {
+#pragma unroll
+            for (int i = 0; i < 4; ++i) gq[i] = __builtin_elementwise_fma(gelu_f32x2{C[7], C[7]}, gs[i], gelu_f32x2{C[6], C[6]});
+#pragma unroll
+            for (int i = 0; i < 4; ++i) gq[i] = __builtin_elementwise_fma(gq[i], gs[i], gelu_f32x2{C[5], C[5]});
+        } else if (st == 3 || st == 4) {
+#pragma unroll
+            for (int k = 0; k < 2; ++k)
+#pragma unroll
+                for (int i = 0; i < 4; ++i) gq[i] = __builtin_elementwise_fma(gq[i], gs[i], gelu_f32x2{C[10 - 2 * st - k], C[10 - 2 * st - k]});
+        } else if (st == 5) {
+#pragma unroll
+            for (int i = 0; i < 4; ++i) gq[i] = __builtin_elementwise_fma(gq[i], gs[i], gelu_f32x2{C[0], C[0]});
+#pragma unroll
+            for (int i = 0; i < 4; ++i) gq[i] = gc[i] * gq[i];
+        } else if (st == 6) {
+            bf16x8 hb;
+#pragma unroll
+            for (int i = 0; i < 4; ++i) {
+                gv[i] = __builtin_elementwise_fma(gv[i], gq[i], gv[i]);
+                hb[2 * i] = (__bf16)gv[i].x; hb[2 * i + 1] = (__bf16)gv[i].y;
+            }
+            hbv = __builtin_bit_cast(u32x4q, hb);
+        } else {
+            Lx[(size_t)((sg + XP) & 1) * (XBYTES / 16) + (wv * 4 + 2 * tt + b) * 64 + lane] = hbv;
+            if (m + 1 < GM) gelu_b1(sg, b ^ 1);
+        }
+    };
+    auto phase_b = [&](int s, auto last_c) {
+        constexpr bool LAST = decltype(last_c)::value;
+        [[maybe_unused]] const bool nl = s + 2 == NST;
         if constexpr (LAST) {
 #pragma unroll
             for (int tt = 0; tt < 2; ++tt)
 #pragma unroll
                 for (int j = 0; j < 4; ++j)
                     xq[tt][j] = __builtin_bit_cast(u32x4q, __builtin_amdgcn_raw_buffer_load_b128(xsrc, (int)(base + (32u * tt + 8u * j + ot) * RB + 128u * wv + ob), 0, 0));
+        } else {
+            gelu_b1(s + 1, 0);
         }
         const u32x4q* const Lr = Lx + (size_t)((s + XP) & 1) * (XBYTES / 16) + lane;
         u32x4q hq[2][2][2];
@@ -735,20 +796,49 @@
             }
 #pragma unroll
             for (int j = 0; j < 4; ++j) {
-                const int i = KS1 + 4 * hl + j, c2 = j & 1, q = j >> 1;
+                const int i = 4 * hl + j, c2 = j & 1, q = j >> 1;
                 const bf16x8 a = __builtin_bit_cast(bf16x8, ring[i % RD]);
-                if (i + RD < NF) ring[i % RD] = frag(s, i + RD);
-                else if (!LAST) ring[i % RD] = frag(sn, i + RD - NF);
+                if (i + RD < 4 * SH) ring[i % RD] = w2f(s, i + RD);
+                else if (!LAST) {
+                    const int n = i + RD - 4 * SH;
+                    ring[i % RD] = wf(nl ? SH * (s + 1) + (n >> 2) : SH * (s + 2) + wv, nl ? KS1 + 4 * wv + 2 * (n & 1) + ((n >> 1) & 1) : n);
+                }
                 d2[c2][0] = __builtin_amdgcn_mfma_f32_32x32x16_bf16(a, __builtin_bit_cast(bf16x8, hq[hl & 1][0][q]), d2[c2][0], 0, 0, 0);
                 d2[c2][1] = __builtin_amdgcn_mfma_f32_32x32x16_bf16(a, __builtin_bit_cast(bf16x8, hq[hl & 1][1][q]), d2[c2][1], 0, 0, 0);
+                if constexpr (!LAST) {
+#pragma unroll
+                    for (int p = 0; p < (GM + 4 * SH - 1) / (4 * SH); ++p)
+                        if (i * GM / (4 * SH) + p < (i + 1) * GM / (4 * SH)) gelu_piece(s + 1, i * GM / (4 * SH) + p);
+                }
                 __builtin_amdgcn_sched_barrier(0);
             }
         }
     };
+    phase_a(0, std::true_type{});
+    RCX_MLP_STAMP(1)
+    gelu_b1(0, 0);
+#pragma unroll
+    for (int m = 0; m < GM; ++m) gelu_piece(0, m);
+    __builtin_amdgcn_s_waitcnt(LGKM0);
+    RCX_MLP_STAMP(2)
+    __builtin_amdgcn_s_barrier();
+    RCX_MLP_STAMP(4)
 #pragma unroll 1
-    for (int s = 0; s < NST - 1; ++s) step(s, std::false_type{});
-    step(NST - 1, std::true_type{});
+    for (int s = 0; s < NST - 1; ++s) {
+        RCX_MLP_STAMP_STEP
+        phase_a(s + 1, std::false_type{});
+        RCX_MLP_STAMP(1)
+        phase_b(s, std::false_type{});
+        __builtin_amdgcn_s_waitcnt(LGKM0);
+        RCX_MLP_STAMP(3)
+        __builtin_amdgcn_s_barrier();
+        RCX_MLP_STAMP(4)
+    }
+    RCX_MLP_STAMP_STEP
+    phase_b(NST - 1, std::true_type{});
+    RCX_MLP_STAMP(3)
     unsigned char* const Lt = lds_raw + (size_t)wv * L::IMG;
+    [[maybe_unused]] float pool_sum = 0.f;
 #pragma unroll
     for (int tt = 0; tt < 2; ++tt) {
 #pragma unroll
@@ -760,10 +850,27 @@
         for (int j = 0; j < 4; ++j) {
             const unsigned char* src = Lt + (8 * j + ot) * OP + 2 * ob;
             const f32x4q lo = *reinterpret_cast<const f32x4q*>(src), hi = *reinterpret_cast<const f32x4q*>(src + 16);
-            __builtin_amdgcn_raw_buffer_store_b128(__builtin_bit_cast(u32x4q, rows_plus_x(lo, hi, xq[tt][j])), ysrc, (int)(base + (32u * tt + 8u * j + ot) * RB + 128u * wv + ob), 0, 0);
+            const bf16x8 o = rows_plus_x(lo, hi, xq[tt][j]);
+            __builtin_amdgcn_raw_buffer_store_b128(__builtin_bit_cast(u32x4q, o), ysrc, (int)(base + (32u * tt + 8u * j + ot) * RB + 128u * wv + ob), 0, 0);
+            if constexpr (POOL) {
+                *reinterpret_cast<f32x4q*>(Lt + (8 * j + ot) * OP + 2 * ob) = f32x4q{(float)o[0], (float)o[1], (float)o[2], (float)o[3]};
+                *reinterpret_cast<f32x4q*>(Lt + (8 * j + ot) * OP + 2 * ob + 16) = f32x4q{(float)o[4], (float)o[5], (float)o[6], (float)o[7]};
+            }
         }
         wave_sync();
-    }
+        if constexpr (POOL) {
+            const int rows = P - 32 * tt < 32 ? P - 32 * tt : 32;
+            float pv[32];
+#pragma unroll
+            for (int t = 0; t < 32; ++t) pv[t] = *reinterpret_cast<const float*>(Lt + t * OP + 4 * lane);
+#pragma unroll
+            for (int t = 0; t < 32; ++t) pool_sum = t < rows ? pool_sum + pv[t] : pool_sum;
+            wave_sync();
+        }
+    }
+    if constexpr (POOL) pooled[(size_t)blockIdx.x * (16 * KS1) + 64 * wv + lane] = f32_to_bf16(pool_sum * (1.0f / (float)P));
+    RCX_MLP_STAMP(5)
+    RCX_MLP_STAMP_END((int)blockIdx.x * NW + wv)
 }
 
 }
@@ -865,17 +972,34 @@
     if (C != CH) return hipErrorInvalidConfiguration;
     auto kfn = mlp::k_channel_mlp_wide<KS1, HT, CT, 8, NW>;
     RCX_SET_LDS_ONCE(kfn, L::bytes);
-    hipLaunchKernelGGL(kfn, dim3((unsigned)((M + 63) / 64)), dim3(64 * NW), L::bytes, s, (const bf16_t*)z, (const bf16_t*)x, (bf16_t*)y, (const mlp::u32x4q*)wfrag, bias, M);
+    hipLaunchKernelGGL(kfn, dim3((unsigned)((M + 63) / 64)), dim3(64 * NW), L::bytes, s, (const bf16_t*)z, (const bf16_t*)x, (bf16_t*)y, (const mlp::u32x4q*)wfrag, bias, M,
+                       (bf16_t*)nullptr, 0 RCX_MLP_STAMP_VAL);
     return hipGetLastError();
 }
 
-struct MlpRow { int C, HT, min_tokens; mlp_launcher launch; };
+#define RCX_MLP_POOL_ARGS const void* z, const void* x, void* y, void* pooled, const void* wfrag, const float* bias, int N, int P, int C, hipStream_t s
+typedef hipError_t (*mlp_pool_launcher)(RCX_MLP_POOL_ARGS);
+template <int CH, int HT>
+static hipError_t launch_mlp_wide_pool(RCX_MLP_POOL_ARGS)
+{
+    constexpr int KS1 = mlp_ks1(CH), CT = mlp_ct(CH), NW = CT / 2;
+    using L = mlp::WideLds<KS1, HT, CT, NW>;
+    static_assert(CH == 16 * KS1 && CH == 64 * NW, "no padding lanes; a wave's 64 lanes own its 64 output channels");
+    if (C != CH || N <= 0 || P <= 0 || P > 64) return hipErrorInvalidConfiguration;
+    auto kfn = mlp::k_channel_mlp_wide<KS1, HT, CT, 8, NW, true>;
+    RCX_SET_LDS_ONCE(kfn, L::bytes);
+    hipLaunchKernelGGL(kfn, dim3((unsigned)N), dim3(64 * NW), L::bytes, s, (const bf16_t*)z, (const bf16_t*)x, (bf16_t*)y, (const mlp::u32x4q*)wfrag, bias, N * P,
+                       (bf16_t*)pooled, P RCX_MLP_STAMP_VAL);
+    return hipGetLastError();
+}
+
+struct MlpRow { int C, HT, min_tokens; mlp_launcher launch; mlp_pool_launcher pool = nullptr; };
 static constexpr MlpRow MLP_ROWS[] = {
     {256, 16, 1, launch_mlp_pair<256, 16>},
     {128, 8, 1, launch_mlp_res128<128, 8>},
-    {512, 32, 2048, launch_mlp_wide<512, 32>},
-    {512, 24, 512, launch_mlp_wide<512, 24>},
-    {384, 24, 784, launch_mlp_wide<384, 24>},
+    {512, 32, 2048, launch_mlp_wide<512, 32>, launch_mlp_wide_pool<512, 32>},
+    {512, 24, 512, launch_mlp_wide<512, 24>, launch_mlp_wide_pool<512, 24>},
+    {384, 24, 784, launch_mlp_wide<384, 24>, launch_mlp_wide_pool<384, 24>},
     {192, 12, 1, launch_mlp_stream<192, 12>},
     {160, 10, 1, launch_mlp_stream<160, 10>},
     {320, 20, 1, launch_mlp_stream<320, 20, 2, false>},
@@ -915,6 +1039,19 @@
     return row->launch(z, x, y, wfrag, bias, M, C, ncu, s);
 }
 
+bool channel_mlp_pool_applicable(int N, int P, int C, int H, int dtype)
+{
+    if (opt::off(opt::MLP_POOL) || N <= 0 || P <= 0 || P > 64 || N > (1 << 24)) return false;
+    const MlpRow* const row = mlp_row(N * P, C, H, dtype);
+    return row && row->pool;
+}
+
+hipError_t channel_mlp_pool(const void* z, const void* x, void* y, void* pooled, const void* wfrag, const float* bias, int N, int P, int C, int H, int dtype, hipStream_t s)
+{
+    if (!channel_mlp_pool_applicable(N, P, C, H, dtype)) return hipErrorInvalidConfiguration;
+    return mlp_row(N * P, C, H, dtype)->pool(z, x, y, pooled, wfrag, bias, N, P, C, s);
+}
+
 }
 
 #ifdef RCX_MLP_STAMPS
diff --git a/recnext_amd/csrc/rcx_opts.h b/recnext_amd/csrc/rcx_opts.h
--- a/recnext_amd/csrc/rcx_opts.h
+++ b/recnext_amd/csrc/rcx_opts.h
@@ -6,13 +6,13 @@
 namespace rcx {
 namespace opt {
 
-enum Id { FORCE_GENERIC, CPL, CPL14, CPL14_RL, CPT, CPT_CB, CPT16, UPADD_CPL, UPADD_CPT, NESTED, TRAIN_FUSED, BWD_FUSED, WGRAD_CPL, COUNT };
+enum Id { FORCE_GENERIC, CPL, CPL14, CPL14_RL, CPT, CPT_CB, CPT16, UPADD_CPL, UPADD_CPT, NESTED, TRAIN_FUSED, BWD_FUSED, WGRAD_CPL, MLP_POOL, COUNT };
 
 namespace detail {
 inline const char* name_of(int i)
 {
     static const char* const k[COUNT] = {"RCX_FORCE_GENERIC", "RCX_CPL", "RCX_CPL14", "RCX_CPL14_RL", "RCX_CPT", "RCX_CPT_CB", "RCX_CPT16",
-                                         "RCX_UPADD_CPL", "RCX_UPADD_CPT", "RCX_NESTED", "RCX_TRAIN_FUSED", "RCX_BWD_FUSED", "RCX_WGRAD_CPL"};
+                                         "RCX_UPADD_CPL", "RCX_UPADD_CPT", "RCX_NESTED", "RCX_TRAIN_FUSED", "RCX_BWD_FUSED", "RCX_WGRAD_CPL", "RCX_MLP_POOL"};
     return k[i];
 }
 struct Table {
diff --git a/recnext_amd/layers.py b/recnext_amd/layers.py
--- a/recnext_amd/layers.py
+++ b/recnext_amd/layers.py
@@ -122,6 +122,12 @@
     def __init__(self, fc1, fc2):
         self.fc1, self.fc2 = fc1, fc2
         self._key, self._pack = None, None
+        self.feeds_pool = False
+        self._pooled = None
+
+    def take_pooled(self, y):
+        held, self._pooled = self._pooled, None
+        return held[1] if held is not None and held[0] is y else None
 
     def supported(self, x):
         from . import ops
@@ -153,6 +159,11 @@
         from . import ops
         n, c, h, w = x.shape
         wfrag, bias, hidden = self._operands(ops.channel_mlp_hidden(n * h * w, c, self.fc1.out_channels, x.dtype))
+        self._pooled = None
+        if self.feeds_pool and ops.channel_mlp_pool_supported(n, h * w, c, hidden, x.dtype):
+            y, pooled = ops.channel_mlp(z, x, wfrag, bias, hidden, pool=True)
+            self._pooled = (y, pooled)
+            return y
         return ops.channel_mlp(z, x, wfrag, bias, hidden)
 
 
diff --git a/recnext_amd/models.py b/recnext_amd/models.py
--- a/recnext_amd/models.py
+++ b/recnext_amd/models.py
@@ -160,8 +160,17 @@
 
     def forward_head(self, x):
         if self.global_pool == "avg":
-            x = x.mean((2, 3))
+            pooled = self._pooled_by_last_block(x)
+            x = pooled if pooled is not None else x.mean((2, 3))
         return self.head(self.head_drop(x))
+
+    def _pooled_by_last_block(self, x):
+        if self.training or x.dtype != torch.bfloat16 or len(self.stages) == 0:
+            return None
+        blocks = getattr(self.stages[-1], "blocks", None)
+        last = blocks[-1] if blocks is not None and len(blocks) else None
+        fused = last.__dict__.get("_fused_mlp") if last is not None else None
+        return fused.take_pooled(x) if fused is not None else None
 
     def forward(self, x):
         return self.forward_head(self.forward_features(x))
@@ -299,6 +308,10 @@
                     and getattr(seq[1], "approximate", "none") == "none":
                 object.__setattr__(m, "_fused_mlp", FusedChannelMlp(seq[0], seq[2]))
                 n += 1
+    if isinstance(net, RecNext) and net.global_pool == "avg" and len(net.stages) and len(net.stages[-1].blocks):
+        fused = net.stages[-1].blocks[-1].__dict__.get("_fused_mlp")
+        if fused is not None:
+            fused.feeds_pool = True
     return n
 
 
diff --git a/recnext_amd/ops.py b/recnext_amd/ops.py
--- a/recnext_amd/ops.py
+++ b/recnext_amd/ops.py
@@ -646,7 +646,7 @@
         raise ValueError(f"{name} must be a contiguous {dtype} tensor of {numel} elements on {device}, got {got}")
 
 
-def channel_mlp(z, x, wfrag, bias, hidden):
+def channel_mlp(z, x, wfrag, bias, hidden, pool=False):
     z = _nhwc(z, "z")
     x = _nhwc(x, "x")
     if z.shape != x.shape or z.dtype != x.dtype:
@@ -660,10 +660,23 @@
     if z.device != x.device:
         raise ValueError("z and x must be on the same device")
     y = _empty_nhwc(n, c, h, w, x.dtype, x.device)
+    if pool:
+        pooled = torch.empty((n, c), dtype=x.dtype, device=x.device)
+        with _on(x.device):
+            rc = lib.rcx_channel_mlp_pool_fwd(z.data_ptr(), x.data_ptr(), y.data_ptr(), pooled.data_ptr(), wfrag.data_ptr(), bias.data_ptr(), n, h * w, c, hidden, _dt(x),
+                                              _stream(x.device))
+        _lib.check(rc, "rcx_channel_mlp_pool_fwd")
+        return y, pooled
     with _on(x.device):
         rc = lib.rcx_channel_mlp_fwd(z.data_ptr(), x.data_ptr(), y.data_ptr(), wfrag.data_ptr(), bias.data_ptr(), n * h * w, c, hidden, _dt(x), _stream(x.device))
     _lib.check(rc, "rcx_channel_mlp_fwd")
     return y
+
+
+def channel_mlp_pool_supported(n, p, c, hidden, dtype):
+    if dtype != torch.bfloat16 or hidden <= 0:
+        return False
+    return _lib.load().rcx_channel_mlp_pool_supported(int(n), int(p), int(c), int(hidden), _DT[dtype]) > 0
 
 
 def stem_supported(n, h, w, cm, co, dtype):
```

Result: no change. 119,800 (median of 6 runs) (+0.7%).
